# NilanEkanayake/TiTok-Video

Measured on AMD Instinct MI355X. Metric: video clips/sec encode+decode (whole node), higher is better.
Workload: dtype bf16

## Files before the change

include/titok_hip.h:

```cpp
#ifndef TITOK_HIP_H
#define TITOK_HIP_H

#include <stdint.h>

#ifdef __cplusplus
extern "C" {
#endif

#define TTV_OK 0
#define TTV_ERR_INVALID 1
#define TTV_ERR_LAUNCH 2
#define TTV_ERR_UNSUPPORTED 3

#define TTV_BF16 0
#define TTV_F32 1

#define TTV_ENCODER 0
#define TTV_DECODER 1

#define TTV_MAX_FSQ 8
#define TTV_MAX_TOKEN 64
#define TTV_MAX_CLIPS_PER_LAUNCH 64

const char* ttv_error_string(void);
// ... 50 lines not shown

int ttv_rmsnorm(const void* in, int in_dtype, int ld_in, const int32_t* src_rows, void* out, int out_dtype, int ld_out,
                const int32_t* dst_rows, const float* gain, int rows, int width, float eps, void* stream);

int ttv_rope_apply(void* x, int dtype, int ld, int rows, int heads, const float* rope_cs, void* stream);

int ttv_linear(const void* x, int ldx, const void* w, int ldw, const void* bias, const float* add_scalar, void* y, int ldy,
               int M, int N, int K, int dtype, void* stream);

int ttv_linear_qkv_rope(const void* x, int ldx, const void* w, int ldw, void* y, int ldy, int M, int d_model, int gqa_dim,
                        const float* rope_cs, int dtype, void* stream);
int ttv_linear_geglu(const void* x, int ldx, const void* w, int ldw, void* y, int ldy, int M, int I, int K, int dtype,
                     void* stream);
int ttv_linear_residual(const void* x, int ldx, const void* w, int ldw, const void* resid, int ldr, float alpha, void* y,
                        int ldy, int y_f32, int M, int N, int K, int dtype, void* stream);

int ttv_linear_residual_norm(const void* x, int ldx, const void* w, int ldw, const void* resid, int ldr, float alpha,
                             const float* gain, float eps, void* y, int ldy, int M, int N, int K, int dtype, void* stream);

int64_t ttv_mlp_pack_bytes(int inner, int next_qkv_rows);
int ttv_mlp_pack(const void* w12_folded, const void* w3, const void* out_proj, const void* next_qkv_folded, int next_qkv_rows, int inner,
                 int width, int dtype, void* mlp_packed, void* stream);
int ttv_mlp_fused(const void* x, int ldx, const void* mlp_packed, int inner, void* y, int ldy, const float* post_gain, float alpha,
                  float eps, int M, int width, int dtype, void* stream);
typedef struct ttv_next_qkv {
  void* qkv; int32_t ld;
  const float* rope_cs;
  int32_t rows;
  int32_t rope_q_end, rope_k_begin, rope_k_end;
} ttv_next_qkv;
int ttv_layer_tail_fused(const void* ao, int ldao, const float* attn_post_gain, float attn_alpha, const void* x, int ldx,
                         const void* mlp_packed, int inner, void* y, int ldy, const float* ffd_post_gain, float ffd_alpha, float eps,
                         int M, int width, int dtype, const ttv_next_qkv* next, void* stream);

int ttv_fill_const_rows(void* x, int dtype, int ld, const int32_t* rows_map, int rows, int width, const float* mask_token,
                        const float* gain, float eps, void* stream);
int ttv_decoder_embed(const void* codes, int token_size, const void* w, const void* bias, const float* mask_token, const float* gain,
                      void* x, int dtype, int ld, const int32_t* rows_map, int rows, int width, float eps, void* stream);

#define TTV_ATTN_GATE 1
#define TTV_ATTN_PAIRED 2
#define TTV_ATTN_QSCALED 4
#define TTV_ATTN_ALLFULL 8
#define TTV_ATTN_PIPE 16
#define TTV_ATTN_SPLIT3 32
#define TTV_ATTN_SPLIT_OUT 64
#define TTV_ATTN_SPLIT_IN 128
int ttv_attention(const void* qkvg, int ld, void* out, int ldo, const int32_t* cu_seqlens, const int32_t* qblocks,
                  int n_qblocks, int q_heads, int kv_heads, int head_dim, int flags, int dtype, void* stream);
int ttv_attention64(const void* qkvg, int ld, void* out, int ldo, const int32_t* cu_seqlens, const int32_t* items, int n_items,
                    int q_heads, int kv_heads, int head_dim, int flags, int dtype, void* stream);

int ttv_rmsnorm_mx(const void* in, int in_dtype, int ld_in, void* out, int out_dtype, int ld_out, const float* gain, int rows, int width,
                   float eps, float* next_rstd, void* mx_q, void* mx_s, void* stream);
int ttv_attention_mxout(const void* qkvg, int ld, void* out_q, void* out_mx, int ld_mx, const int32_t* cu_seqlens, const int32_t* qblocks,
                        int n_qblocks, int q_heads, int kv_heads, void* stream);
int ttv_linear_fp8_mx_geglu_q(const void* xq, int ldx, const void* x_mx, const float* x_row_scale, const void* wq, int ldw, const void* w_mx,
                              const float* w_row_scale, void* hq, void* hq_mx, int M, int N, int K, void* stream);

int ttv_row_rstd(const void* x, int dtype, int ldx, float* rstd, int rows, int width, float eps, void* stream);
int ttv_linear_rowscale(const void* x, int ldx, const void* w, int ldw, const float* row_scale, int epilogue, const float* rope_cs, int d_model,
                        int gqa_dim, void* y, int ldy, int M, int N, int K, int dtype, void* stream);

int ttv_patch_gather(const void* const* clips, const int32_t* clip_desc, int clip0, int n_clips, int patch_t, int patch_h,
                     int patch_w, int channels, void* patches, int ld, int dtype, int max_patches_per_clip, void* stream);
int ttv_patch_embed_norm(const void* const* clips, const int32_t* clip_desc, const int32_t* patch_rows, const int32_t* row_seq, int n_clips,
                         int patch_t, int patch_h, int patch_w, int channels, const void* w, int ldw, const void* bias,
                         const float* mask_token, const float* gain, float eps, void* x, int ldx, int rows, int width, int dtype,
                         void* stream);
int ttv_patch_scatter(const void* patches, int ld, const int32_t* clip_desc, int clip0, int n_clips, int patch_t, int patch_h,
                      int patch_w, int channels, void* const* clips, int dtype, int max_patches_per_clip, void* stream);
// ... 358 lines not shown
#define TTV_KC_GEMM_RESID 4
#define TTV_KC_GEMM_STORE 5
#define TTV_KC_RMSNORM 6
#define TTV_KC_PATCH 7
#define TTV_KC_ROWS 8
int ttv_prof_begin(int kernel_class, int max_records);
enum {
  TTV_DBG_NO_STORES = 1,
  TTV_DBG_K256_NO_PANEL_DMA = 2,
  TTV_DBG_MLP_NO_WEIGHT_DMA = 2,
  TTV_DBG_K256_NO_TILE_RELOAD = 4,
  TTV_DBG_MLP_NO_GEGLU = 4,
  TTV_DBG_K256_NO_EPILOGUE_MATH = 8,
  TTV_DBG_MLP_TILES8 = 8,
  TTV_DBG_MLP_NO_P2 = 16,
  TTV_DBG_MLP_PAIRS_ONLY = 32,
  TTV_DBG_MLP_TILES4 = 64,
  TTV_DBG_GEMM_TILE160 = 128,
  TTV_DBG_GEMM_TILE128 = 256,
  TTV_DBG_GEMM_T256 = 512,
  TTV_DBG_MLP_TILES9 = 512,
  TTV_DBG_GEMM_NO_T256 = 1024,
  TTV_DBG_MX_UNFUSED_QUANT = 2048,
  TTV_DBG_SPLIT3_NO_IMAGES = 4096,
  TTV_DBG_SPLIT3_NO_DMA = 8192,
  TTV_DBG_K256_GENERAL = 16384,
  TTV_DBG_QKV256_OFF = 32768,
  TTV_DBG_QKV256_WS = 131072,
  TTV_DBG_ENC_ALL_ROWS = 524288,
  TTV_DBG_ATTN_NO_SWP = 1048576,
  TTV_DBG_DEC_ALL_BLOCKS = 2097152,
  TTV_DBG_DEC_L0_NO_CONST = 4194304,
  TTV_DBG_ENC_LAST_QKV_ALL = 8388608,
  TTV_DBG_PATCH_EMBED_UNFUSED = 16777216
};
int ttv_debug_set(int flags);
int ttv_debug_stamps(void* device_buffer);
int ttv_prof_end(double* total_ms, int* count);

#ifdef __cplusplus
}
#endif
#endif
```

titok_video_amd/_lib.py:

```python
from __future__ import annotations

import ctypes as C
import os
import threading

import torch

from . import switches

TTV_BF16, TTV_F32 = 0, 1
TTV_ENCODER, TTV_DECODER = 0, 1
TTV_MAX_FSQ = 8
TTV_MAX_TOKEN = 64
TTV_MAX_CLIPS_PER_LAUNCH = 64
TTV_DISC_HEAD_GENERATOR, TTV_DISC_HEAD_DISCRIMINATOR = 0, 1
TTV_TAPE_STORED, TTV_TAPE_RECOMPUTE = 0, 1

DBG_NO_STORES = 1
DBG_K256_NO_PANEL_DMA = 2
DBG_MLP_NO_WEIGHT_DMA = 2
DBG_K256_NO_TILE_RELOAD = 4
DBG_MLP_NO_GEGLU = 4
DBG_K256_NO_EPILOGUE_MATH = 8
DBG_MLP_TILES8 = 8
DBG_MLP_NO_P2 = 16
DBG_MLP_PAIRS_ONLY = 32
DBG_MLP_TILES4 = 64
DBG_GEMM_TILE160 = 128
DBG_GEMM_TILE128 = 256
DBG_GEMM_T256 = 512
DBG_MLP_TILES9 = 512
DBG_GEMM_NO_T256 = 1024
DBG_MX_UNFUSED_QUANT = 2048
DBG_SPLIT3_NO_IMAGES = 4096
DBG_SPLIT3_NO_DMA = 8192
DBG_K256_GENERAL = 16384
DBG_QKV256_OFF = 32768
DBG_QKV256_WS = 131072
DBG_ENC_ALL_ROWS = 524288
DBG_ATTN_NO_SWP = 1048576
DBG_DEC_ALL_BLOCKS = 2097152
DBG_DEC_L0_NO_CONST = 4194304
DBG_ENC_LAST_QKV_ALL = 8388608
DBG_PATCH_EMBED_UNFUSED = 16777216

_HERE = os.path.dirname(os.path.abspath(__file__))
LIB_PATH = switches.text("TTV_LIB_PATH") or os.path.join(_HERE, "libtitok_hip.so")

i32, i64, f32, vp = C.c_int32, C.c_int64, C.c_float, C.c_void_p


class FsqParams(C.Structure):
    _fields_ = [("n", i32), ("levels", i32 * TTV_MAX_FSQ), ("basis", i32 * TTV_MAX_FSQ),
                ("half_l", f32 * TTV_MAX_FSQ), ("offset", f32 * TTV_MAX_FSQ), ("shift", f32 * TTV_MAX_FSQ),
                ("half_width", f32 * TTV_MAX_FSQ)]


class TowerDims(C.Structure):
    _fields_ = [("kind", i32), ("dtype", i32), ("width", i32), ("layers", i32), ("q_heads", i32), ("kv_heads", i32),
                ("head_dim", i32), ("inner", i32), ("patch_t", i32), ("patch_h", i32), ("patch_w", i32),
                ("pix_channels", i32), ("token_size", i32), ("eps", f32), ("alpha", f32)]


class NextQkv(C.Structure):
    _fields_ = [("qkv", vp), ("ld", i32), ("rope_cs", vp), ("rows", i32), ("rope_q_end", i32), ("rope_k_begin", i32), ("rope_k_end", i32)]


class LayerWeights(C.Structure):
    _fields_ = [("pre_ln", vp), ("to_qkv", vp), ("out_proj", vp), ("ffd_norm", vp), ("w12", vp), ("w3", vp),
                ("attn_post_ln", vp), ("ffd_post_ln", vp), ("to_qkv_pn", vp), ("w12_pn", vp), ("mlp_pack", vp), ("mlp_pack_qkv_rows", i32), ("qkv_q_prescaled", i32),
                ("to_qkv_qs", vp), ("to_qkv_f8", vp), ("to_qkv_f8_scale", vp), ("w12_f8", vp), ("w12_f8_scale", vp),
                ("to_qkv_mx", vp), ("w12_mx", vp), ("out_proj_f8", vp), ("out_proj_f8_scale", vp), ("out_proj_mx", vp),
                ("w3_f8", vp), ("w3_f8_scale", vp), ("w3_mx", vp)]


class TowerWeights(C.Structure):
    _fields_ = [("proj_in_w", vp), ("proj_in_b", vp), ("mask_token", vp), ("ln_pre_t", vp), ("ln_pre_p", vp),
# ... 99 lines not shown
    "ttv_fsq_forward": (C.c_int, [C.POINTER(FsqParams), vp, C.c_int, C.c_int, vp, C.c_int, vp, vp, vp]),
    "ttv_fsq_indices_to_codes": (C.c_int, [C.POINTER(FsqParams), vp, C.c_int, vp, C.c_int, vp]),
    "ttv_vq_codebook_norms": (C.c_int, [vp, C.c_int, C.c_int, C.c_int, C.c_int, vp, vp]),
    "ttv_vq_workspace_bytes": (C.c_int64, [C.c_int]),
    "ttv_vq_l2_argmin": (C.c_int, [vp, C.c_int, C.c_int, vp, C.c_int, vp, C.c_int, C.c_int, C.c_int, vp, vp, vp, C.c_int64, vp]),
    "ttv_vq_lookup": (C.c_int, [vp, C.c_int, C.c_int, vp, C.c_int, C.c_int, vp, C.c_int, vp]),
    "ttv_vq_lookup_backward": (C.c_int, [vp, C.c_int, C.c_int, vp, C.c_int, C.c_int, vp, C.c_int, vp]),
    "ttv_vq_train_workspace_bytes": (C.c_int64, [C.c_int, C.c_int]),
    "ttv_vq_commit_forward": (C.c_int, [vp, C.c_int, C.c_int, vp, C.c_int, vp, C.c_int, C.c_int, C.c_int, vp, vp, C.c_int64, vp]),
    "ttv_vq_commit_backward": (C.c_int, [vp, C.c_int, vp, C.c_int, vp, C.c_int, C.c_int, C.c_int, C.c_int, C.c_double, vp, C.c_int, vp]),
    "ttv_vq_ema_stats": (C.c_int, [vp, C.c_int, C.c_int, vp, C.c_int, C.c_int, C.c_int, vp, f32, C.c_uint64, vp, C.c_int, C.c_int, vp, vp, C.c_int64, vp]),
    "ttv_vq_ema_update": (C.c_int, [vp, vp, vp, vp, vp, C.c_int, vp, vp, C.c_int, C.c_int, f32, f32, f32, f32, vp, C.c_int64, vp]),
    "ttv_quant_rows_fp8": (C.c_int, [vp, C.c_int, C.c_int, vp, f32, vp, C.c_int, vp, C.c_int, C.c_int, vp]),
    "ttv_linear_fp8": (C.c_int, [vp, C.c_int, vp, vp, C.c_int, vp, vp, C.c_int, C.c_int, C.c_int, C.c_int, C.c_int, vp, C.c_int, C.c_int, vp]),
    "ttv_split3_pack": (C.c_int, [vp, C.c_int, vp, C.c_int, C.c_int, C.c_int, vp]),
    "ttv_linear_split3": (C.c_int, [vp, C.c_int, vp, C.c_int, vp, vp, C.c_int, C.c_int, C.c_int, C.c_int, vp]),
    "ttv_mx_scale_bytes_per_row": (C.c_int64, [C.c_int]),
    "ttv_quant_mx_fp8": (C.c_int, [vp, C.c_int, C.c_int, vp, C.c_int, vp, vp, C.c_int, C.c_int, vp]),
    "ttv_linear_fp8_mx": (C.c_int, [vp, C.c_int, vp, vp, vp, C.c_int, vp, vp, vp, C.c_int, C.c_int, C.c_int, C.c_int, C.c_int, vp, C.c_int, C.c_int,
                                    vp, C.c_int, f32, vp]),
    "ttv_rmsnorm": (C.c_int, [vp, C.c_int, C.c_int, vp, vp, C.c_int, C.c_int, vp, vp, C.c_int, C.c_int, f32, vp]),
    "ttv_rope_apply": (C.c_int, [vp, C.c_int, C.c_int, C.c_int, C.c_int, vp, vp]),
    "ttv_linear": (C.c_int, [vp, C.c_int, vp, C.c_int, vp, vp, vp, C.c_int, C.c_int, C.c_int, C.c_int, C.c_int, vp]),
    "ttv_linear_qkv_rope": (C.c_int, [vp, C.c_int, vp, C.c_int, vp, C.c_int, C.c_int, C.c_int, C.c_int, vp, C.c_int, vp]),
    "ttv_linear_geglu": (C.c_int, [vp, C.c_int, vp, C.c_int, vp, C.c_int, C.c_int, C.c_int, C.c_int, C.c_int, vp]),
    "ttv_linear_residual": (C.c_int, [vp, C.c_int, vp, C.c_int, vp, C.c_int, f32, vp, C.c_int, C.c_int, C.c_int, C.c_int,
                                      C.c_int, C.c_int, vp]),
    "ttv_linear_residual_norm": (C.c_int, [vp, C.c_int, vp, C.c_int, vp, C.c_int, f32, vp, f32, vp, C.c_int, C.c_int, C.c_int,
                                           C.c_int, C.c_int, vp]),
    "ttv_mlp_pack_bytes": (C.c_int64, [C.c_int, C.c_int]),
    "ttv_mlp_pack": (C.c_int, [vp, vp, vp, vp, C.c_int, C.c_int, C.c_int, C.c_int, vp, vp]),
    "ttv_layer_tail_fused": (C.c_int, [vp, C.c_int, vp, f32, vp, C.c_int, vp, C.c_int, vp, C.c_int, vp, f32, f32, C.c_int, C.c_int,
                                       C.c_int, vp, vp]),
    "ttv_mlp_fused": (C.c_int, [vp, C.c_int, vp, C.c_int, vp, C.c_int, vp, f32, f32, C.c_int, C.c_int, C.c_int, vp]),
    "ttv_fill_const_rows": (C.c_int, [vp, C.c_int, C.c_int, vp, C.c_int, C.c_int, vp, vp, f32, vp]),
    "ttv_decoder_embed": (C.c_int, [vp, C.c_int, vp, vp, vp, vp, vp, C.c_int, C.c_int, vp, C.c_int, C.c_int, f32, vp]),
    "ttv_attention": (C.c_int, [vp, C.c_int, vp, C.c_int, vp, vp, C.c_int, C.c_int, C.c_int, C.c_int, C.c_int, C.c_int, vp]),
    "ttv_attention64": (C.c_int, [vp, C.c_int, vp, C.c_int, vp, vp, C.c_int, C.c_int, C.c_int, C.c_int, C.c_int, C.c_int, vp]),
    "ttv_rmsnorm_mx": (C.c_int, [vp, C.c_int, C.c_int, vp, C.c_int, C.c_int, vp, C.c_int, C.c_int, f32, vp, vp, vp, vp]),
    "ttv_attention_mxout": (C.c_int, [vp, C.c_int, vp, vp, C.c_int, vp, vp, C.c_int, C.c_int, C.c_int, vp]),
    "ttv_linear_fp8_mx_geglu_q": (C.c_int, [vp, C.c_int, vp, vp, vp, C.c_int, vp, vp, vp, vp, C.c_int, C.c_int, C.c_int, vp]),
    "ttv_row_rstd": (C.c_int, [vp, C.c_int, C.c_int, vp, C.c_int, C.c_int, f32, vp]),
    "ttv_linear_rowscale": (C.c_int, [vp, C.c_int, vp, C.c_int, vp, C.c_int, vp, C.c_int, C.c_int, vp, C.c_int, C.c_int, C.c_int, C.c_int, C.c_int, vp]),
    "ttv_patch_gather": (C.c_int, [C.POINTER(vp), vp, C.c_int, C.c_int, C.c_int, C.c_int, C.c_int, C.c_int, vp, C.c_int,
                                   C.c_int, C.c_int, vp]),
    "ttv_patch_embed_norm": (C.c_int, [C.POINTER(vp), vp, vp, vp, C.c_int, C.c_int, C.c_int, C.c_int, C.c_int, vp, C.c_int, vp, vp, vp, f32,
                                       vp, C.c_int, C.c_int, C.c_int, C.c_int, vp]),
    "ttv_patch_scatter": (C.c_int, [vp, C.c_int, vp, C.c_int, C.c_int, C.c_int, C.c_int, C.c_int, C.c_int, C.POINTER(vp),
                                    C.c_int, C.c_int, vp]),
    "ttv_tower_workspace_bytes": (i64, [C.POINTER(TowerDims), C.POINTER(Batch)]),
    "ttv_encoder_forward": (C.c_int, [C.POINTER(TowerDims), C.POINTER(TowerWeights), C.POINTER(Batch), C.POINTER(vp),
                                      C.POINTER(FsqParams), vp, vp, vp, vp, vp, i64, vp]),
    "ttv_decoder_forward": (C.c_int, [C.POINTER(TowerDims), C.POINTER(TowerWeights), C.POINTER(Batch), vp, C.POINTER(vp),
                                      vp, i64, vp]),
    "ttv_dec_l0_const_bytes": (i64, [C.POINTER(TowerDims), C.c_int]),
    "ttv_dec_l0_const_build": (C.c_int, [C.POINTER(TowerDims), C.POINTER(TowerWeights), vp, vp, vp, vp, C.c_int, vp, i64, C.POINTER(i64), C.POINTER(i64), vp]),
    "ttv_decoder_forward_const": (C.c_int, [C.POINTER(TowerDims), C.POINTER(TowerWeights), C.POINTER(Batch), vp, C.POINTER(vp),
                                            vp, i64, C.POINTER(DecL0Const), vp]),
    "ttv_tower_tape_bytes": (i64, [C.POINTER(TowerDims), C.POINTER(Batch)]),
    "ttv_tower_bwd_workspace_bytes": (i64, [C.POINTER(TowerDims), C.POINTER(Batch)]),
    "ttv_encoder_forward_train": (C.c_int, [C.POINTER(TowerDims), C.POINTER(TowerWeights), C.POINTER(Batch), C.POINTER(vp), vp, vp,
                                            i64, vp]),
    "ttv_encoder_backward": (C.c_int, [C.POINTER(TowerDims), C.POINTER(TowerWeights), C.POINTER(TowerWeightsT), C.POINTER(Batch), vp,
                                       vp, C.POINTER(TowerGrads), C.POINTER(vp), vp, i64, vp]),
    "ttv_decoder_forward_train": (C.c_int, [C.POINTER(TowerDims), C.POINTER(TowerWeights), C.POINTER(Batch), vp, C.POINTER(vp), vp,
                                            i64, vp, i64, vp]),
    "ttv_decoder_backward": (C.c_int, [C.POINTER(TowerDims), C.POINTER(TowerWeights), C.POINTER(TowerWeightsT), C.POINTER(Batch), vp,
                                       C.POINTER(vp), vp, C.POINTER(TowerGrads), vp, vp, i64, vp]),
    "ttv_tower_tape_bytes_ex": (i64, [C.POINTER(TowerDims), C.POINTER(Batch), C.c_int]),
# ... 127 lines not shown
```

titok_video_amd/csrc/ttv_api.hip:

```cpp
#include <stdarg.h>
#include <stdio.h>
#include <stdlib.h>
#include <string.h>

#include "ttv_common.h"
#include "ttv_kernels.h"

static thread_local char g_err[512] = "";

void ttv_set_error(const char* fmt, ...) {
  va_list ap;
  va_start(ap, fmt);
  vsnprintf(g_err, sizeof(g_err), fmt, ap);
  va_end(ap);
}

int g_ttv_prof_class = 0;
bool ttv_sw_enc_latent_last() { static const bool v = ttv_env_flag("TTV_ENC_LATENT_LAST", true); return v; }
bool ttv_enc_latent_rows_only(const ttv_tower_dims* d, const ttv_batch* b) {
  return ttv_sw_enc_latent_last() && !(g_ttv_debug & TTV_DBG_ENC_ALL_ROWS) && d->kind == TTV_ENCODER && b->latent_rows && b->sum_tokens > 0 &&
         b->sum_tokens < b->total_rows;
}
bool ttv_sw_keel_f32sum() { static const bool v = ttv_env_flag("TTV_KEEL_F32SUM", false); return v; }
bool ttv_sw_fused_patch() { static const bool v = ttv_env_flag("TTV_FUSED_PATCH", true); return v; }
bool ttv_sw_attn_pipe() { static const bool v = ttv_env_flag("TTV_ATTN_PIPE", false); return v; }
static bool sw_dec_l0_const() { static const bool v = ttv_env_flag("TTV_DEC_L0_CONST", true); return v; }
static bool sw_enc_last_qkv_skip() { static const bool v = ttv_env_flag("TTV_ENC_LAST_QKV_SKIP", true); return v; }
float ttv_sw_attn_thr() { static const float v = ttv_env_float("TTV_ATTN_THR", 8.0f); return v; }
thread_local int g_ttv_debug = 0;
long long* g_ttv_stamps = nullptr;
static hipEvent_t* g_prof_start = nullptr;
static hipEvent_t* g_prof_stop = nullptr;
static int g_prof_cap = 0, g_prof_n = 0;

TtvProfScope::TtvProfScope(int cls, hipStream_t stream) : slot(-1), s(stream) {
  if (g_ttv_prof_class != 0 && cls == g_ttv_prof_class && g_prof_n < g_prof_cap) {
    slot = g_prof_n++;
    (void)hipEventRecord(g_prof_start[slot], s);
  }
}
TtvProfScope::~TtvProfScope() {
  if (slot >= 0) (void)hipEventRecord(g_prof_stop[slot], s);
}

struct TowerWs {
  char *x, *xn, *qkv, *ao, *h, *pa, *pb;
  char *xl, *aol;
  char *f8, *f8mx;
  float* y32;
  float* rstd;
  int64_t total;
};

static TowerWs carve(const ttv_tower_dims* d, const ttv_batch* b, char* base) {
  const int64_t e = dtype_bytes(d->dtype);
  const int64_t L = b->total_rows, P = b->sum_patches;
  const int64_t g = (int64_t)d->kv_heads * d->head_dim;
  const int64_t pd = patch_dim(d);
  int64_t off = 0;
  TowerWs w;
// ... 74 lines not shown
    TTV_TRY(ttvk_rmsnorm(ws.x, dt, dm, nullptr, ws.x, dt, dm, nullptr, lw.attn_post_ln, L, dm, d->eps, s, ws.rstd, fused_q ? ws.f8 : nullptr,
                         fused_q ? ws.f8mx : nullptr));
    if (!fused_q) TTV_TRY(ttvk_quant_mx_fp8(ws.x, dt, dm, ws.f8, dm, ws.f8mx, nullptr, L, dm, s));
  } else {
    TTV_TRY(ttvk_row_rstd(ws.x, dt, dm, ws.rstd, L, dm, d->eps, s));
    TTV_TRY(ttvk_quant_mx_fp8(ws.x, dt, dm, ws.f8, dm, ws.f8mx, nullptr, L, dm, s));
  }
  GemmArgs f = gemm_args(dt, ws.f8, dm, lw.w12_f8, dm, L, I, dm, ws.h, I);
  char* const hq = ws.h;
  char* const hq_mx = ws.xn;
  const bool h_fused = fused_q && (int64_t)ttvk_mx_scale_ld(I) <= (int64_t)dm * 2;
  if (h_fused) { f.yq = hq; f.yq_mx = hq_mx; }
  TTV_TRY(ttvk_gemm_fp8(EPI_GEGLU, f, ws.rstd, lw.w12_f8_scale, s, ws.f8mx, lw.w12_mx));
  if (!h_fused) TTV_TRY(ttvk_quant_mx_fp8(ws.h, dt, I, ws.f8, I, ws.f8mx, nullptr, L, I, s));
  const GemmArgs f3 = gemm_resid(gemm_args(dt, h_fused ? hq : ws.f8, I, lw.w3_f8, I, L, dm, I, ws.x, dm), ws.x, dm, alpha);
  TTV_TRY(ttvk_gemm_fp8(EPI_RESID_T, f3, nullptr, lw.w3_f8_scale, s, h_fused ? hq_mx : ws.f8mx, lw.w3_mx));
  rstd_valid = false;
  if (i > 0) {
    TTV_TRY(ttvk_rmsnorm(ws.x, dt, dm, nullptr, ws.x, dt, dm, nullptr, lw.ffd_post_ln, L, dm, d->eps, s, ws.rstd, fused_q ? ws.f8 : nullptr,
                         fused_q ? ws.f8mx : nullptr));
    rstd_valid = true;
    xq_valid = fused_q;
  }
  return TTV_OK;
}

static bool rows_f8(int dt, int dm, const void* img, const void* row_scale, const void* mx, const void* folded) {
  return dt == TTV_BF16 && img && row_scale && !mx && dm % 128 == 0 && !(dm == 256 && folded);
}

struct PreNormW { const float* gain; const void *w, *w_pn, *w_f8; const float* w_f8_scale; bool f8; };

static int prenorm_proj(const LayerCtx& c, GemmEpilogue epi, const char* x, int rows, const PreNormW& p, int N, char* y, int y_image,
                        bool rstd_valid, int tile_run = 0, int tile_period = 0, int panel_lo = 0) {
  const ttv_tower_dims* d = c.d;
  const TowerWs& ws = c.ws;
  const int dm = d->width, dt = d->dtype;
  GemmArgs a = gemm_args(dt, nullptr, dm, nullptr, dm, rows, N, dm, y, N);
  if (epi == EPI_QKV_ROPE) a = gemm_rope_qk(a, c.b->rope_cs, dm, d->kv_heads * d->head_dim);
  if (p.f8) {
    float* const f8_scales = reinterpret_cast<float*>(ws.xn + align256((int64_t)c.b->total_rows * dm));
    TTV_TRY(ttvk_quant_rows_fp8(x, dt, dm, p.gain, d->eps, ws.xn, dm, f8_scales, rows, dm, c.s));
    a.x = ws.xn; a.w = p.w_f8;
    return ttvk_gemm_fp8(epi, a, f8_scales, p.w_f8_scale, c.s);
  }
  const bool fold256 = dt == TTV_BF16 && dm == 256 && p.w_pn;
  const bool fold_gen = c.gen_ok && p.w_pn;
  const bool fold = fold256 || fold_gen;
  if (fold_gen && !rstd_valid) TTV_TRY(ttvk_row_rstd(x, dt, dm, ws.rstd, rows, dm, d->eps, c.s));
  if (!fold) TTV_TRY(ttvk_rmsnorm(x, dt, dm, nullptr, ws.xn, dt, dm, nullptr, p.gain, rows, dm, d->eps, c.s, nullptr, nullptr, nullptr, c.s3img));
  a.split3 = c.split3; a.x_image = c.s3img && !fold; a.y_image = y_image;
  a.prenorm = fold256; a.eps = d->eps;
  a.row_scale = fold_gen ? ws.rstd : nullptr;
  a.x = fold ? x : ws.xn; a.w = fold ? p.w_pn : p.w;
  if (epi == EPI_QKV_ROPE) { a.rope_ids = c.b->rope_ids; a.rope_base = c.b->rope_ids ? c.b->rope_base : nullptr; }
  a.tile_run = tile_run; a.tile_period = tile_period; a.panel_lo = panel_lo;
  return ttvk_gemm(epi, a, c.s);
}

static int keel_tail(const LayerCtx& c, GemmArgs o, int layer, const float* post_gain, bool want_rstd, bool& rstd_valid) {
  const ttv_tower_dims* d = c.d;
  const int dm = d->width, dt = d->dtype;
  char* const cx = (char*)o.y;
  o = gemm_resid(o, cx, dm, keel_alpha(d, layer));
  o.split3 = c.split3; o.x_image = c.s3img;
  if (layer == 0) return ttvk_gemm(EPI_RESID_T, o, c.s);
  if (ttvk_gemm_supports_resid_norm(dt, dm, o.K)) {
    o.norm_gain = post_gain; o.eps = d->eps;
    return ttvk_gemm(EPI_RESID_NORM, o, c.s);
  }
  float* const next_rstd = want_rstd ? c.ws.rstd : nullptr;
  if (dt == TTV_BF16 && !ttv_sw_keel_f32sum()) {
    TTV_TRY(ttvk_gemm(EPI_RESID_T, o, c.s));
    TTV_TRY(ttvk_rmsnorm(cx, dt, dm, nullptr, cx, dt, dm, nullptr, post_gain, o.M, dm, d->eps, c.s, next_rstd));
  } else {
    o.y = c.ws.y32;
    TTV_TRY(ttvk_gemm(EPI_RESID_F32, o, c.s));
    TTV_TRY(ttvk_rmsnorm(c.ws.y32, TTV_F32, dm, nullptr, cx, dt, dm, nullptr, post_gain, o.M, dm, d->eps, c.s, next_rstd));
  }
  rstd_valid = want_rstd;
  return TTV_OK;
}

static bool qkv_tile_list_ok(const LayerCtx& c, const ttv_layer_weights& lw, int K, int P) {
  const ttv_tower_dims* d = c.d;
  const ttv_batch* b = c.b;
  if (d->dtype != TTV_BF16 || d->width != 256 || d->head_dim != 64 || c.split3) return false;
  if (K <= 0 || P <= 0 || K % 128 || P % 128 || (int64_t)b->n_clips * K != b->sum_tokens || (int64_t)b->n_clips * P != b->sum_patches) return false;
  if (!lw.to_qkv_pn || !lw.qkv_q_prescaled) return false;
  return ttvk_gemm_qkv_tiles_supported(d->width, d->kv_heads * d->head_dim, d->width);
}

static bool dec_l0_const_ok(const LayerCtx& c, const ttv_tower_weights* w, const ttv_dec_l0_const* l0) {
  const ttv_tower_dims* d = c.d;
  const ttv_batch* b = c.b;
  if (!l0 || !l0->rows || !sw_dec_l0_const() || (g_ttv_debug & TTV_DBG_DEC_L0_NO_CONST)) return false;
  if (d->kind != TTV_DECODER || !qkv_tile_list_ok(c, w->layers[0], l0->latent_rows, l0->patch_rows)) return false;
  if (c.pair || c.pipe || !c.all_full || (b->items64 && b->n_items64 > 0)) return false;
  return ttvk_attention_takes_swp(TTV_ATTN_GATE | TTV_ATTN_QSCALED | TTV_ATTN_ALLFULL);
}

static bool enc_last_qkv_skip_ok(const LayerCtx& c, const ttv_layer_weights& lw) {
  const ttv_batch* b = c.b;
  if (!sw_enc_last_qkv_skip() || (g_ttv_debug & TTV_DBG_ENC_LAST_QKV_ALL) || c.d->kind != TTV_ENCODER) return false;
  return qkv_tile_list_ok(c, lw, b->tokens_per_clip, b->max_patches_per_clip);
}

static int run_layers(const ttv_tower_dims* d, const ttv_tower_weights* w, const ttv_batch* b, const TowerWs& ws, hipStream_t s,
                      const ttv_dec_l0_const* l0 = nullptr) {
  const int L = b->total_rows, dm = d->width, g = d->kv_heads * d->head_dim, dt = d->dtype;
  const int split3 = (dt == TTV_F32 && w->f32_split3) ? 1 : 0;
  const bool gen_ok = (dt == TTV_BF16 && dm != 256) || split3;
  static const bool s3img_env = ttv_env_flag("TTV_SPLIT3_IMAGES", true);
  const int s3img = (split3 && s3img_env && !(g_ttv_debug & TTV_DBG_SPLIT3_NO_IMAGES)) ? 1 : 0;
  const int nq = 2 * dm + 2 * g;
  const int64_t row_bytes = (int64_t)dm * dtype_bytes(dt);
  bool qkv_ready = false;
  bool rstd_valid = false;
  bool xq_valid = false;
  const bool lat_last = ttv_enc_latent_rows_only(d, b) && b->qblocks_latent && b->n_qblocks_latent > 0;
  static const bool pat_env = ttv_env_flag("TTV_DEC_PATCH_LAST", true);
  const bool pat_last = pat_env && !(g_ttv_debug & TTV_DBG_DEC_ALL_BLOCKS) && d->kind == TTV_DECODER && d->layers >= 2 && b->qblocks_patch &&
                        b->n_qblocks_patch > 0 && !split3 && !b->qblocks_paired;
  bool compacted = false;
  const LayerCtx ctx = {d, b, ws, s, split3, s3img, gen_ok, b->qblocks_paired ? TTV_ATTN_PAIRED : 0, b->qblocks_all_full ? TTV_ATTN_ALLFULL : 0,
                        ttv_sw_attn_pipe() ? TTV_ATTN_PIPE : 0};
  const bool l0_const = dec_l0_const_ok(ctx, w, l0);
  for (int i = 0; i < d->layers; ++i) {
    const ttv_layer_weights& lw = w->layers[i];
    const bool last = i == d->layers - 1;
    const bool l0c = l0_const && i == 0;
    if (dt == TTV_BF16 && dm != 256 && dm % 128 == 0 && d->inner % 128 == 0 && !ttv_sw_keel_f32sum() && lw.to_qkv_f8 && lw.to_qkv_mx && lw.w12_f8 &&
        lw.w12_mx && lw.out_proj_f8 && lw.out_proj_mx && lw.w3_f8 && lw.w3_mx &&
        !(lat_last && last)) {
      TTV_TRY(run_layer_mx(ctx, lw, i, rstd_valid, xq_valid));
      qkv_ready = false;
      continue;
    }
    xq_valid = false;
    const bool f8_qkv = rows_f8(dt, dm, lw.to_qkv_f8, lw.to_qkv_f8_scale, lw.to_qkv_mx, lw.to_qkv_pn);
    const bool f8_w12 = rows_f8(dt, dm, lw.w12_f8, lw.w12_f8_scale, lw.w12_mx, lw.w12_pn);
    if (!qkv_ready) {
      const void* w_plain = (dt == TTV_BF16 && lw.to_qkv_qs) ? lw.to_qkv_qs : lw.to_qkv;
      const PreNormW qw = {lw.pre_ln, w_plain, lw.to_qkv_pn, lw.to_qkv_f8, lw.to_qkv_f8_scale, f8_qkv};
      if (l0c) TTV_TRY(prenorm_proj(ctx, EPI_QKV_ROPE, ws.x, L, qw, nq, ws.qkv, 0, rstd_valid, l0->latent_rows / 128, (l0->latent_rows + l0->patch_rows) / 128));
      else if (lat_last && last && !f8_qkv && enc_last_qkv_skip_ok(ctx, lw))
        TTV_TRY(prenorm_proj(ctx, EPI_QKV_ROPE, ws.x, L, qw, nq, ws.qkv, 0, rstd_valid, b->tokens_per_clip / 128,
                             (b->tokens_per_clip + b->max_patches_per_clip) / 128, 2 * dm / 64));
      else TTV_TRY(prenorm_proj(ctx, EPI_QKV_ROPE, ws.x, L, qw, nq, ws.qkv, s3img ? 2 : 0, rstd_valid));
    }
    const bool q_scaled = dt == TTV_BF16 && (lw.to_qkv_pn ? lw.qkv_q_prescaled != 0 : lw.to_qkv_qs != nullptr);
    rstd_valid = false;
    qkv_ready = false;
    const bool lat_now = lat_last && last;
    if (lat_now)
      TTV_TRY(tower_attention(ctx, q_scaled, b->qblocks_latent, b->n_qblocks_latent, ctx.all_full));
    else if (l0c) {
      TtvProfScope prof(TTV_KC_ATTENTION, s);
      const bool own = l0->qblocks && l0->n_qblocks > 0;
      TTV_TRY(ttvk_attention_swp(ws.qkv, nq, ws.ao, dm, b->cu_seqlens, own ? l0->qblocks : b->qblocks, own ? l0->n_qblocks : b->n_qblocks, d->q_heads,
                                 d->kv_heads, 1, s, l0->rows, l0->latent_rows, l0->state));
    } else if (pat_last && last && dt == TTV_BF16 && !ctx.pipe)
      TTV_TRY(tower_attention(ctx, q_scaled, b->qblocks_patch, b->n_qblocks_patch, ctx.all_full));
    else if (q_scaled && b->items64 && b->n_items64 > 0 && d->head_dim == 64)
      TTV_TRY(ttvk_attention64(ws.qkv, nq, ws.ao, dm, b->cu_seqlens, b->items64, b->n_items64, d->q_heads, d->kv_heads,
                               TTV_ATTN_GATE | TTV_ATTN_QSCALED, s));
    else
      TTV_TRY(tower_attention(ctx, q_scaled, b->qblocks, b->n_qblocks, ctx.pair | ctx.all_full | ctx.pipe));
    char* cx = ws.x;
    char* cao = ws.ao;
    int Lc = L;
    if (lat_now) {
      TTV_TRY(gather_rows(ws.x, ws.xl, b->latent_rows, b->sum_tokens, row_bytes, s));
      TTV_TRY(gather_rows(ws.ao, ws.aol, b->latent_rows, b->sum_tokens, row_bytes, s));
      cx = ws.xl; cao = ws.aol; Lc = b->sum_tokens;
      compacted = true;
    }
    static const bool use_fused_mlp = ttv_env_flag("TTV_FUSED_MLP", true);
    static const bool use_fused_qkv = ttv_env_flag("TTV_FUSED_QKV", false);
    const float alpha = keel_alpha(d, i);
    if (use_fused_mlp && ttvk_mlp_fused_supported(dt, dm, d->inner) && lw.mlp_pack) {
      MlpNextQkv nx = {};
      const bool back = use_fused_qkv && !last && lw.mlp_pack_qkv_rows == nq && nq % 64 == 0 && dm % 64 == 0 && g % 64 == 0;
      if (back) { nx.qkv = ws.qkv; nx.ld = nq; nx.rope_cs = b->rope_cs; nx.rows = nq; nx.rope_q_end = dm; nx.rope_k_begin = 2 * dm; nx.rope_k_end = 2 * dm + g; }
      TTV_TRY(ttvk_mlp_fused(cao, dm, i == 0 ? nullptr : lw.attn_post_ln, alpha, cx, dm, lw.mlp_pack, d->inner, cx, dm, i == 0 ? nullptr : lw.ffd_post_ln,
                             alpha, d->eps, Lc, back ? &nx : nullptr, s));
      qkv_ready = back;
      continue;
    }
    TTV_TRY(keel_tail(ctx, gemm_args(dt, cao, dm, lw.out_proj, dm, Lc, dm, dm, cx, dm), i, lw.attn_post_ln, gen_ok && lw.w12_pn && !f8_w12, rstd_valid));
    const PreNormW fw = {lw.ffd_norm, lw.w12, lw.w12_pn, lw.w12_f8, lw.w12_f8_scale, f8_w12};
    TTV_TRY(prenorm_proj(ctx, EPI_GEGLU, cx, Lc, fw, d->inner, ws.h, s3img, rstd_valid));
    rstd_valid = false;
    const ttv_layer_weights* nl = last ? nullptr : &w->layers[i + 1];
    const bool next_rstd = gen_ok && nl && nl->to_qkv_pn && !rows_f8(dt, dm, nl->to_qkv_f8, nl->to_qkv_f8_scale, nl->to_qkv_mx, nl->to_qkv_pn);
    TTV_TRY(keel_tail(ctx, gemm_args(dt, ws.h, d->inner, lw.w3, d->inner, Lc, dm, d->inner, cx, dm), i, lw.ffd_post_ln, next_rstd, rstd_valid));
  }
  if (compacted)
    TTV_TRY(scatter_rows(ws.xl, ws.x, b->latent_rows, b->sum_tokens, row_bytes, s));
  return TTV_OK;
}

static bool fused_patch_ok(const ttv_tower_dims* d, const ttv_batch* b, int dt) {
  auto pow2 = [](int v) { return v > 0 && (v & (v - 1)) == 0; };
  return ttv_sw_fused_patch() && dt == TTV_BF16 && d->patch_w == 8 && pow2(d->patch_t) && pow2(d->patch_h) &&
         b->n_clips <= TTV_MAX_CLIPS_PER_LAUNCH && b->row_seq && patch_dim(d) % 64 == 0;
}

extern "C" {

const char* ttv_error_string(void) { return g_err; }
int ttv_version(void) { return 100; }

int ttv_fsq_forward(const ttv_fsq_params* p, const void* z, int z_dtype, int rows, void* codes, int codes_dtype, int32_t* indices,
                    float* bounded, void* stream) {
  TTV_CHECK_ARG(rows >= 0 && (rows == 0 || (z && codes && indices)), "fsq_forward: null buffer");
  return ttvk_fsq_forward(p, z, z_dtype, rows, codes, codes_dtype, indices, bounded, (hipStream_t)stream);
}

// ... 169 lines not shown
int ttv_mlp_pack(const void* w12_folded, const void* w3, const void* out_proj, const void* next_qkv_folded, int next_qkv_rows, int inner,
                 int width, int dtype, void* packed, void* stream) {
  if (!ttvk_mlp_fused_supported(dtype, width, inner)) {
    ttv_set_error("mlp_pack: only bf16, width 256, inner %% 32 == 0");
    return TTV_ERR_UNSUPPORTED;
  }
  return ttvk_mlp_pack(w12_folded, w3, out_proj, next_qkv_folded, next_qkv_rows, inner, packed, (hipStream_t)stream);
}

int ttv_mlp_fused(const void* x, int ldx, const void* mlp_packed, int inner, void* y, int ldy, const float* post_gain, float alpha,
                  float eps, int M, int width, int dtype, void* stream) {
  if (!ttvk_mlp_fused_supported(dtype, width, inner)) {
    ttv_set_error("mlp_fused: only bf16, width 256, inner %% 32 == 0");
    return TTV_ERR_UNSUPPORTED;
  }
  return ttvk_mlp_fused(nullptr, 0, nullptr, 1.f, x, ldx, mlp_packed, inner, y, ldy, post_gain, alpha, eps, M, nullptr, (hipStream_t)stream);
}

int ttv_layer_tail_fused(const void* ao, int ldao, const float* attn_post_gain, float attn_alpha, const void* x, int ldx,
                         const void* mlp_packed, int inner, void* y, int ldy, const float* ffd_post_gain, float ffd_alpha, float eps,
                         int M, int width, int dtype, const ttv_next_qkv* next, void* stream) {
  if (!ttvk_mlp_fused_supported(dtype, width, inner)) {
    ttv_set_error("layer_tail_fused: only bf16, width 256, inner %% 32 == 0");
    return TTV_ERR_UNSUPPORTED;
  }
  TTV_CHECK_ARG(ao, "layer_tail_fused: null attention output");
  MlpNextQkv nx = {};
  if (next) { nx.qkv = next->qkv; nx.ld = next->ld; nx.rope_cs = next->rope_cs; nx.rows = next->rows; nx.rope_q_end = next->rope_q_end;
              nx.rope_k_begin = next->rope_k_begin; nx.rope_k_end = next->rope_k_end; }
  return ttvk_mlp_fused(ao, ldao, attn_post_gain, attn_alpha, x, ldx, mlp_packed, inner, y, ldy, ffd_post_gain, ffd_alpha, eps, M,
                        next ? &nx : nullptr, (hipStream_t)stream);
}

int ttv_fill_const_rows(void* x, int dtype, int ld, const int32_t* rows_map, int rows, int width, const float* mask_token,
                        const float* gain, float eps, void* stream) {
  TTV_CHECK_ARG(rows == 0 || (x && rows_map && mask_token && gain), "fill_const_rows: null buffer");
  return ttvk_fill_const_rows(x, dtype, ld, rows_map, rows, width, mask_token, gain, eps, (hipStream_t)stream);
}

int ttv_decoder_embed(const void* codes, int token_size, const void* w, const void* bias, const float* mask_token, const float* gain,
                      void* x, int dtype, int ld, const int32_t* rows_map, int rows, int width, float eps, void* stream) {
  TTV_CHECK_ARG(rows == 0 || (codes && w && bias && mask_token && gain && x && rows_map), "decoder_embed: null buffer");
  return ttvk_dec_embed(codes, token_size, w, bias, mask_token, gain, x, dtype, ld, rows_map, rows, width, eps, (hipStream_t)stream);
}

int ttv_attention(const void* qkvg, int ld, void* out, int ldo, const int32_t* cu_seqlens, const int32_t* qblocks, int n_qblocks,
                  int q_heads, int kv_heads, int head_dim, int flags, int dtype, void* stream) {
  TTV_CHECK_ARG(n_qblocks == 0 || (qkvg && out && cu_seqlens && qblocks), "attention: null buffer");
  return ttvk_attention(qkvg, ld, out, ldo, cu_seqlens, qblocks, n_qblocks, q_heads, kv_heads, head_dim, flags, dtype, (hipStream_t)stream);
}
int ttv_attention64(const void* qkvg, int ld, void* out, int ldo, const int32_t* cu_seqlens, const int32_t* items, int n_items, int q_heads,
                    int kv_heads, int head_dim, int flags, int dtype, void* stream) {
  TTV_CHECK_ARG(dtype == TTV_BF16 && head_dim == 64, "attention64: bf16, head_dim 64 only");
  return ttvk_attention64(qkvg, ld, out, ldo, cu_seqlens, items, n_items, q_heads, kv_heads, flags, (hipStream_t)stream);
}

int ttv_rmsnorm_mx(const void* in, int in_dtype, int ld_in, void* out, int out_dtype, int ld_out, const float* gain, int rows, int width,
                   float eps, float* next_rstd, void* mx_q, void* mx_s, void* stream) {
  TTV_CHECK_ARG(rows >= 0 && (rows == 0 || (in && out && gain)), "rmsnorm_mx: null buffer");
  TTV_CHECK_ARG(!mx_q == !mx_s, "rmsnorm_mx: the image needs both its element and its scale buffer");
  return ttvk_rmsnorm(in, in_dtype, ld_in, nullptr, out, out_dtype, ld_out, nullptr, gain, rows, width, eps, (hipStream_t)stream, next_rstd, mx_q, mx_s);
}

int ttv_attention_mxout(const void* qkvg, int ld, void* out_q, void* out_mx, int ld_mx, const int32_t* cu_seqlens, const int32_t* qblocks,
                        int n_qblocks, int q_heads, int kv_heads, void* stream) {
  TTV_CHECK_ARG(n_qblocks >= 0 && (n_qblocks == 0 || (qkvg && out_q && out_mx && cu_seqlens && qblocks)), "attention_mxout: null buffer");
  return ttvk_attention_mxout(qkvg, ld, out_q, out_mx, ld_mx, cu_seqlens, qblocks, n_qblocks, q_heads, kv_heads, (hipStream_t)stream);
}

int ttv_linear_fp8_mx_geglu_q(const void* xq, int ldx, const void* x_mx, const float* x_row_scale, const void* wq, int ldw, const void* w_mx,
                              const float* w_row_scale, void* hq, void* hq_mx, int M, int N, int K, void* stream) {
  TTV_CHECK_ARG(M == 0 || (xq && wq && x_mx && w_mx && hq && hq_mx), "linear_fp8_mx_geglu_q: null buffer");
  GemmArgs a = gemm_args(TTV_BF16, xq, ldx, wq, ldw, M, N, K, hq, N);
  a.yq = hq; a.yq_mx = hq_mx;
  return ttvk_gemm_fp8(EPI_GEGLU, a, x_row_scale, w_row_scale, (hipStream_t)stream, x_mx, w_mx);
}
// ... 116 lines not shown
  char* const rows = (char*)block;
  const int64_t state_floats = ttvk_attention_swp_state_floats(patch_rows, d->q_heads);
  float* const state = (float*)(rows + align256((int64_t)patch_rows * nq * 2));
  char* const x = (char*)state + align256(state_floats * 4 + 4);
  if (state_offset) *state_offset = (char*)state - rows;
  if (flag_offset) *flag_offset = (char*)(state + state_floats) - rows;
  TTV_TRY(ttvk_fill_const_rows(x, dt, dm, iota, patch_rows, dm, w->mask_token, w->ln_pre_p, d->eps, s));
  GemmArgs a = gemm_rope_qk(gemm_args(dt, x, dm, lw.to_qkv_pn, dm, patch_rows, nq, dm, rows, nq), rope_cs, dm, g);
  a.prenorm = 1; a.eps = d->eps;
  a.rope_ids = rope_ids; a.rope_base = rope_ids ? rope_base : nullptr;
  TTV_TRY(ttvk_gemm(EPI_QKV_ROPE, a, s));
  if (hipMemsetAsync(state + state_floats, 0, 4, s) != hipSuccess) {
    ttv_set_error("dec_l0_const_build: hipMemsetAsync failed");
    return TTV_ERR_LAUNCH;
  }
  return ttvk_attention_swp_dump(rows, nq, patch_rows, d->q_heads, d->kv_heads, state, s);
}

int ttv_decoder_forward(const ttv_tower_dims* d, const ttv_tower_weights* w, const ttv_batch* b, const void* codes,
                        void* const* clips_out, void* workspace, int64_t workspace_bytes, void* stream) {
  return ttv_decoder_forward_const(d, w, b, codes, clips_out, workspace, workspace_bytes, nullptr, stream);
}

int ttv_decoder_forward_const(const ttv_tower_dims* d, const ttv_tower_weights* w, const ttv_batch* b, const void* codes,
                              void* const* clips_out, void* workspace, int64_t workspace_bytes, const ttv_dec_l0_const* l0, void* stream) {
  TTV_TRY(check_dims(d, b));
  TTV_CHECK_ARG(d->kind == TTV_DECODER, "decoder_forward: dims.kind is not TTV_DECODER");
  TTV_CHECK_ARG(w && w->layers && codes && clips_out && workspace, "decoder_forward: null argument");
  hipStream_t s = (hipStream_t)stream;
  TowerWs ws = carve(d, b, (char*)workspace);
  TTV_CHECK_ARG(ws.total <= workspace_bytes, "decoder_forward: workspace too small (%lld < %lld)", (long long)workspace_bytes, (long long)ws.total);
  const int dm = d->width, dt = d->dtype, P = b->sum_patches, pd = patch_dim(d);

  TTV_TRY(ttvk_dec_embed(codes, d->token_size, w->proj_in_w, w->proj_in_b, w->mask_token, w->ln_pre_t, ws.x, dt, dm, b->latent_rows, b->sum_tokens, dm, d->eps, s));
  TTV_TRY(ttvk_fill_const_rows(ws.x, dt, dm, b->patch_rows, P, dm, w->mask_token, w->ln_pre_p, d->eps, s));

  TTV_TRY(run_layers(d, w, b, ws, s, l0));

  GemmArgs a = gemm_args(dt, nullptr, dm, w->proj_out_w, dm, P, pd, dm, ws.pa, pd);
  a.split3 = (dt == TTV_F32 && w->f32_split3) ? 1 : 0;
  a.bias = w->proj_out_b;
  if (dt == TTV_BF16 && dm == 256 && w->proj_out_pn && pd % 8 == 0) {
    a.x = ws.x; a.x_rows = b->patch_rows; a.w = w->proj_out_pn; a.prenorm = 1; a.eps = d->eps;
  } else {
    TTV_TRY(ttvk_rmsnorm(ws.x, dt, dm, b->patch_rows, ws.pb, dt, dm, nullptr, w->ln_post, P, dm, d->eps, s));
    a.x = ws.pb;
  }
  if (fused_patch_ok(d, b, dt) && dm == 256) {
    a.clips = clips_out; a.n_clips = b->n_clips; a.clip_desc = b->clip_desc; a.patch_rows = b->patch_rows; a.row_seq = b->row_seq;
    a.patch_t = d->patch_t; a.patch_h = d->patch_h; a.patch_w = d->patch_w;
    return ttvk_gemm(EPI_STORE_PATCH, a, s);
  }
  TTV_TRY(ttvk_gemm(EPI_STORE, a, s));
  return patch_copy_all(true, clips_out, d, b, ws.pa, dt, s);
}

int ttv_rope_table_build(const float* base_cos, const float* base_sin, int n_ids, int n_freqs, const int32_t* clip_desc, const int32_t* cu_seqlens,
                         const int32_t* row_seq, float* rope_cs, int total_rows, void* stream) {
  TTV_CHECK_ARG(total_rows == 0 || (base_cos && base_sin && clip_desc && cu_seqlens && row_seq && rope_cs), "rope_table_build: null buffer");
  TTV_CHECK_ARG(n_freqs >= 1 && 3 * n_freqs <= 32 && n_ids >= 1, "rope_table_build: bad table shape");
  return ttvk_rope_build(base_cos, base_sin, n_ids, n_freqs, clip_desc, cu_seqlens, row_seq, rope_cs, total_rows, (hipStream_t)stream);
}

int ttv_l1_loss(void* const* recon, void* const* target, void* const* grad, const int32_t* sizes, int n_clips, int dtype, float* loss,
                void* stream) {
  return for_clip_groups(n_clips, [&](int c0, int n) {
    return ttvk_l1_loss(recon + c0, target + c0, grad ? grad + c0 : nullptr, sizes + c0, n, n_clips, dtype, loss, (hipStream_t)stream);
  });
// ... 178 lines not shown
```

titok_video_amd/csrc/ttv_elem.hip:

```cpp
#include "ttv_common.h"
#include "ttv_kernels.h"

#define ROWS_PER_BLOCK 4
#define MAX_ITERS 4

__device__ __forceinline__ int mx_quant4(const f32x4 y, int& byte) {
  float a = fmaxf(fmaxf(fabsf(y[0]), fabsf(y[1])), fmaxf(fabsf(y[2]), fabsf(y[3])));
  a = fmaxf(a, __shfl_xor(a, 1));
  a = fmaxf(a, __shfl_xor(a, 2));
  a = fmaxf(a, __shfl_xor(a, 4));
  const uint32_t tb = __float_as_uint(a * (1.0f / 448.0f));
  byte = (int)((tb >> 23) & 0xFF) + ((tb & 0x7FFFFF) ? 1 : 0);
  byte = a > 0.f ? (byte < 1 ? 1 : (byte > 254 ? 254 : byte)) : 127;
  const float inv_blk = __uint_as_float((uint32_t)(254 - byte) << 23);
  int w = 0;
  w = __builtin_amdgcn_cvt_pk_fp8_f32(y[0] * inv_blk, y[1] * inv_blk, w, false);
  w = __builtin_amdgcn_cvt_pk_fp8_f32(y[2] * inv_blk, y[3] * inv_blk, w, true);
  return w;
}

template <typename TI, typename TO>
__global__ __launch_bounds__(256) void k_rmsnorm(const TI* __restrict__ in, int ld_in, const int* __restrict__ src_rows,
                                                 TO* __restrict__ out, int ld_out, const int* __restrict__ dst_rows,
                                                 const float* __restrict__ gain, int rows, int d, float eps,
// ... 305 lines not shown
    a = fmaxf(a, __shfl_xor(a, 2));
    a = fmaxf(a, __shfl_xor(a, 4));
    const uint32_t tb = __float_as_uint(a * (1.0f / 448.0f));
    int byte = (int)((tb >> 23) & 0xFF) + ((tb & 0x7FFFFF) ? 1 : 0);
    byte = a > 0.f ? (byte < 1 ? 1 : (byte > 254 ? 254 : byte)) : 127;
    const float inv_blk = __uint_as_float((uint32_t)(254 - byte) << 23);
    int w = 0;
    w = __builtin_amdgcn_cvt_pk_fp8_f32(y[0] * inv_blk, y[1] * inv_blk, w, false);
    w = __builtin_amdgcn_cvt_pk_fp8_f32(y[2] * inv_blk, y[3] * inv_blk, w, true);
    *reinterpret_cast<int*>(q + c) = w;
    if ((lane & 7) == 0) {
      const int b = c >> 5;
      m[(b & 3) * nkp + (b >> 2)] = (uint8_t)byte;
    }
  }
}

int64_t ttvk_mx_scale_ld(int d) { return 4 * (int64_t)((d / 128 + 3) / 4 * 4); }

int ttvk_quant_mx_fp8(const void* in, int in_dtype, int ld_in, void* out, int ld_out, void* mx, float* row_scales, int rows, int d, hipStream_t s) {
  if (rows == 0) return TTV_OK;
  TTV_CHECK_ARG(d > 0 && d % 128 == 0, "quant_mx_fp8: width %d must be a multiple of 128", d);
  TTV_CHECK_ARG(ld_in % 4 == 0 && ld_out % 4 == 0 && (uintptr_t)out % 4 == 0 && (uintptr_t)mx % 4 == 0, "quant_mx_fp8: alignment");
  const int nkp = (d / 128 + 3) / 4 * 4;
  dim3 grid(ttv_cdiv(rows, ROWS_PER_BLOCK));
  if (in_dtype == TTV_BF16) hipLaunchKernelGGL((k_quant_mx_fp8<bf16_t>), grid, dim3(256), 0, s, (const bf16_t*)in, ld_in, (uint8_t*)out, ld_out, (uint8_t*)mx, 4 * nkp, nkp, row_scales, rows, d);
  else if (in_dtype == TTV_F32) hipLaunchKernelGGL((k_quant_mx_fp8<float>), grid, dim3(256), 0, s, (const float*)in, ld_in, (uint8_t*)out, ld_out, (uint8_t*)mx, 4 * nkp, nkp, row_scales, rows, d);
  else { ttv_set_error("quant_mx_fp8: bad dtype"); return TTV_ERR_INVALID; }
  TTV_CHECK_LAUNCH("quant_mx_fp8");
  return TTV_OK;
}

template <typename T>
__global__ __launch_bounds__(256) void k_fill_const_rows(T* __restrict__ x, int ld, const int* __restrict__ rows_map, int rows,
                                                         int d, const float* __restrict__ mask_token,
                                                         const float* __restrict__ gain, float eps) {
  const int wave = threadIdx.x >> 6, lane = threadIdx.x & 63;
  const int r = blockIdx.x * ROWS_PER_BLOCK + wave;
  if (r >= rows) return;
  const float m = round_to<T>(mask_token[0]);
  const float rstd = 1.0f / sqrtf(m * m + eps);
  T* q = x + (size_t)rows_map[r] * ld;
  for (int c = lane * 4; c < d; c += 256) {
    const f32x4 g = *reinterpret_cast<const f32x4*>(gain + c);
    f32x4 o = {m * rstd * g[0], m * rstd * g[1], m * rstd * g[2], m * rstd * g[3]};
    Vec4<T>::store(q + c, o);
  }
}

int ttvk_fill_const_rows(void* x, int dtype, int ld, const int* rows_map, int rows, int d, const float* mask_token,
                         const float* gain, float eps, hipStream_t s) {
  if (rows == 0) return TTV_OK;
  TTV_CHECK_ARG(d % 4 == 0, "fill_const_rows: width %% 4");
  dim3 grid(ttv_cdiv(rows, ROWS_PER_BLOCK));
  if (dtype == TTV_BF16)
    hipLaunchKernelGGL((k_fill_const_rows<bf16_t>), grid, dim3(256), 0, s, (bf16_t*)x, ld, rows_map, rows, d, mask_token, gain, eps);
  else
    hipLaunchKernelGGL((k_fill_const_rows<float>), grid, dim3(256), 0, s, (float*)x, ld, rows_map, rows, d, mask_token, gain, eps);
  TTV_CHECK_LAUNCH("fill_const_rows");
  return TTV_OK;
}

template <typename T>
__global__ __launch_bounds__(256) void k_dec_embed(const T* __restrict__ codes, int C, const T* __restrict__ w ,
                                                   const T* __restrict__ bias, const float* __restrict__ mask_token,
                                                   const float* __restrict__ gain, T* __restrict__ x, int ld,
                                                   const int* __restrict__ rows_map, int rows, int d, float eps, T* __restrict__ hpre) {
  const int wave = threadIdx.x >> 6, lane = threadIdx.x & 63;
  const int r = blockIdx.x * ROWS_PER_BLOCK + wave;
  if (r >= rows) return;
  float cz[TTV_MAX_FSQ];
#pragma unroll
  for (int c = 0; c < TTV_MAX_FSQ; ++c) cz[c] = c < C ? Cvt<T>::to_f(codes[(size_t)r * C + c]) : 0.f;
  const T* crow = codes + (size_t)r * C;
  const float m = round_to<T>(mask_token[0]);
  float v[MAX_ITERS][4];
  float ss = 0.f;
#pragma unroll
  for (int it = 0; it < MAX_ITERS; ++it) {
#pragma unroll
    for (int e = 0; e < 4; ++e) {
      const int f = (it * 64 + lane) * 4 + e;
      float h = 0.f;
      if (f < d) {
        if (C <= TTV_MAX_FSQ) {
#pragma unroll
          for (int c = 0; c < TTV_MAX_FSQ; ++c)
            if (c < C) h += cz[c] * Cvt<T>::to_f(w[(size_t)f * C + c]);
        } else if ((C & 3) == 0) {
          const T* wrow = w + (size_t)f * C;
          for (int c = 0; c < C; c += 4) {
            const f32x4 cv = Vec4<T>::load(crow + c), wv = Vec4<T>::load(wrow + c);
            h += cv[0] * wv[0];
            h += cv[1] * wv[1];
            h += cv[2] * wv[2];
            h += cv[3] * wv[3];
          }
        } else {
          for (int c = 0; c < C; ++c) h += Cvt<T>::to_f(crow[c]) * Cvt<T>::to_f(w[(size_t)f * C + c]);
        }
        h = round_to<T>(h + Cvt<T>::to_f(bias[f]));
        h = round_to<T>(h + m);
      }
      v[it][e] = h;
      ss += h * h;
    }
    if (hpre && (it * 64 + lane) * 4 < d)
      Vec4<T>::store(hpre + (size_t)r * d + (it * 64 + lane) * 4, (f32x4){v[it][0], v[it][1], v[it][2], v[it][3]});
  }
  ss = wave_sum(ss);
  const float rstd = 1.0f / sqrtf(ss / (float)d + eps);
  T* q = x + (size_t)rows_map[r] * ld;
#pragma unroll
  for (int it = 0; it < MAX_ITERS; ++it) {
    const int c0 = (it * 64 + lane) * 4;
    if (c0 < d) {
      const f32x4 g = *reinterpret_cast<const f32x4*>(gain + c0);
      f32x4 o = {v[it][0] * rstd * g[0], v[it][1] * rstd * g[1], v[it][2] * rstd * g[2], v[it][3] * rstd * g[3]};
      Vec4<T>::store(q + c0, o);
    }
  }
}

int ttvk_dec_embed(const void* codes, int C, const void* w, const void* bias, const float* mask_token, const float* gain,
                   void* x, int dtype, int ld, const int* rows_map, int rows, int d, float eps, hipStream_t s) {
  return ttvk_dec_embed_ex(codes, C, w, bias, mask_token, gain, x, dtype, ld, rows_map, rows, d, eps, nullptr, s);
}

int ttvk_dec_embed_ex(const void* codes, int C, const void* w, const void* bias, const float* mask_token, const float* gain, void* x,
                      int dtype, int ld, const int* rows_map, int rows, int d, float eps, void* hpre, hipStream_t s) {
  if (rows == 0) return TTV_OK;
  TTV_CHECK_ARG(C >= 1 && C <= TTV_MAX_TOKEN, "dec_embed: token_size %d out of range", C);
  TTV_CHECK_ARG(d % 4 == 0 && d <= 1024, "dec_embed: width");
  dim3 grid(ttv_cdiv(rows, ROWS_PER_BLOCK));
  if (dtype == TTV_BF16)
    hipLaunchKernelGGL((k_dec_embed<bf16_t>), grid, dim3(256), 0, s, (const bf16_t*)codes, C, (const bf16_t*)w, (const bf16_t*)bias, mask_token, gain, (bf16_t*)x, ld, rows_map, rows, d, eps, (bf16_t*)hpre);
  else
    hipLaunchKernelGGL((k_dec_embed<float>), grid, dim3(256), 0, s, (const float*)codes, C, (const float*)w, (const float*)bias, mask_token, gain, (float*)x, ld, rows_map, rows, d, eps, (float*)hpre);
  TTV_CHECK_LAUNCH("dec_embed");
  return TTV_OK;
}

struct FsqDev {
  int n;
  float half_l[TTV_MAX_FSQ], offset[TTV_MAX_FSQ], shift[TTV_MAX_FSQ], half_width[TTV_MAX_FSQ], basis[TTV_MAX_FSQ];
  int levels[TTV_MAX_FSQ], ibasis[TTV_MAX_FSQ];
};

static FsqDev to_dev(const ttv_fsq_params* p) {
  FsqDev d;
  d.n = p->n;
  for (int i = 0; i < TTV_MAX_FSQ; ++i) {
    d.half_l[i] = p->half_l[i]; d.offset[i] = p->offset[i]; d.shift[i] = p->shift[i];
    d.half_width[i] = p->half_width[i]; d.basis[i] = (float)p->basis[i];
// ... 357 lines not shown
```

titok_video_amd/csrc/ttv_gemm.hip:

```cpp
#include <stdlib.h>

#include "ttv_common.h"
#include "ttv_kernels.h"

struct GemmDev {
  const void* x; const void* w; void* y;
  const void* bias; const float* add_scalar; const void* resid; const float* rope_cs;
  int ldx, ldw, ldy, ldr;
  int M, N, K;
  int w_rows;
  float alpha;
  int rope_q_end, rope_k_begin, rope_k_end;
  float eps;
  int debug;
  const float* norm_gain;
  ClipPtrs clips;
  const int* clip_desc; const int* patch_rows; const int* row_seq;
  const int* x_rows;
  const float* row_scale;
  const int* rope_ids; const float* rope_base;
  const float* x_scale; const float* w_scale;
  float* sum_f32; int ld_sum;
  void* y2; int ldy2; const float* norm_gain2;
  int split3;
  int x_image, y_image;
  const uint8_t* x_mx; const uint8_t* w_mx;
  int ld_mx;
  uint8_t* yq; uint8_t* yq_mx; int ld_yq_mx, yq_nkp;
  int clip0, pt_shift, ph_shift;
  long long* stamps;
  int resid_rows;
  int tile_run, tile_period;
  int panel_lo;
};

struct PatchDst {
  bf16_t* base;
  int thw, hw, w;
};

__device__ __forceinline__ float gelu_erf(float v) { return 0.5f * v * (1.0f + erff(v * 0.70710678118654752440f)); }
__device__ __forceinline__ float gelu_erf_as(float v) {
  const float x = fabsf(v) * 0.70710678118654752440f;
  const float t = __builtin_amdgcn_rcpf(fmaf(0.3275911f, x, 1.0f));
  const float poly = t * fmaf(t, fmaf(t, fmaf(t, fmaf(t, 1.061405429f, -1.453152027f), 1.421413741f), -0.284496736f), 0.254829592f);
  const float e = __builtin_amdgcn_exp2f(x * x * -1.44269504088896340736f);
  const float erf_abs = fmaf(-poly, e, 1.0f);
  return 0.5f * v * (1.0f + __builtin_copysignf(erf_abs, v));
}

__device__ __forceinline__ uint2 pack_bf16x4(f32x4 v) {
  bf16x4 b = {(bf16_t)v[0], (bf16_t)v[1], (bf16_t)v[2], (bf16_t)v[3]};
  return __builtin_bit_cast(uint2, b);
}

__device__ __forceinline__ uint4 split4_bf16(uint4 v) {
  const float x0 = __uint_as_float(v.x), x1 = __uint_as_float(v.y), x2 = __uint_as_float(v.z), x3 = __uint_as_float(v.w);
  const bf16_t h0 = (bf16_t)x0, h1 = (bf16_t)x1, h2 = (bf16_t)x2, h3 = (bf16_t)x3;
  const bf16_t l0 = (bf16_t)(x0 - (float)h0), l1 = (bf16_t)(x1 - (float)h1), l2 = (bf16_t)(x2 - (float)h2), l3 = (bf16_t)(x3 - (float)h3);
  const bf16x4 hv = {h0, h1, h2, h3}, lv = {l0, l1, l2, l3};
  const uint2 hp = __builtin_bit_cast(uint2, hv), lp = __builtin_bit_cast(uint2, lv);
  return make_uint4(hp.x, hp.y, lp.x, lp.y);
}

template <int EPI, typename T, int NI, int NJ>
__device__ __forceinline__ void epilogue_tile(const GemmDev& p, const int (&tok)[NJ], const int (&feat)[NI],
// ... 1761 lines not shown
    for (int i = 0; i < 2; ++i) {
      feat[i] = fbase + wf * 32 + i * 16 + kq * 4;
#pragma unroll
      for (int j = 0; j < NJ; ++j) { ax[i][j] = acc[i][j]; ag[i][j] = acc[i + 2][j]; }
    }
    epilogue_tile<EPI, float, 2, NJ>(p, tok, feat, ax, ag, kq);
  } else {
    int feat[4];
#pragma unroll
    for (int i = 0; i < 4; ++i) feat[i] = fbase + wf * 64 + i * 16 + kq * 4;
    epilogue_tile<EPI, float, 4, NJ>(p, tok, feat, acc, acc, kq);
  }
}

static int gemm_token_tile(int M, int nf, int debug) {
  if (debug & TTV_DBG_GEMM_TILE160) return 160;
  if (debug & TTV_DBG_GEMM_TILE128) return 128;
  const long cost128 = (long)ttv_cdiv(nf * ttv_cdiv(M, 128), 512) * 128, cost160 = (long)ttv_cdiv(nf * ttv_cdiv(M, 160), 512) * 160;
  return cost160 < cost128 ? 160 : 128;
}

static int sw_qkv256() { static const int v = ttv_env_int("TTV_QKV256", 1); return v; }
bool ttvk_gemm_qkv_tiles_supported(int d_model, int gqa_dim, int ldw) {
  const int N = 2 * d_model + 2 * gqa_dim;
  return sw_qkv256() == 1 && !(g_ttv_debug & (TTV_DBG_QKV256_OFF | TTV_DBG_QKV256_WS)) && N % 64 == 0 && d_model % 64 == 0 && gqa_dim % 64 == 0 &&
         (uint64_t)N * (uint64_t)ldw * 2u < (1ull << 32);
}

template <int EPI>
static int launch(const GemmDev& d, int dtype, bool prenorm, hipStream_t s) {
  if (dtype == TTV_BF16 && d.K == 256 && d.N % 8 == 0 && !((d.debug & TTV_DBG_K256_GENERAL) && !prenorm && EPI != EPI_STORE_PATCH)) {
    const int fo = (EPI == EPI_GEGLU) ? 32 : 64;
    const int n_panels = ttv_cdiv(d.N, fo), n_tiles = d.tile_period ? d.M / K256_TT / d.tile_period * d.tile_run : ttv_cdiv(d.M, K256_TT);
    const int total = n_panels * n_tiles + (d.panel_lo ? d.M / K256_TT / d.tile_period * (d.tile_period - d.tile_run) * (n_panels - d.panel_lo) : 0);
    static const int grid_env = ttv_env_int("TTV_K256_GRID", 0);
    int grid = total < 512 ? total : 512;
    if (grid_env > 0) grid = total < grid_env ? total : grid_env;
    else if (d.panel_lo && total > 512) {
      const int w = n_panels - d.panel_lo;
      for (int ipb = 2; ipb <= w; ++ipb)
        if (w % ipb == 0 && n_panels % ipb == 0 && total / ipb <= 512) { grid = total / ipb; break; }
    } else if (total > 512)
      for (int g = 512; g >= 416; --g)
        if (total % g == 0) { grid = g; break; }
    const int qkv256_env = sw_qkv256();
    if constexpr (EPI == EPI_QKV_ROPE) {
      const int n_groups = (n_panels + 3) / 4;
      if (qkv256_env && !(d.debug & TTV_DBG_QKV256_OFF) && d.N % 64 == 0 && d.rope_q_end % 64 == 0 && d.rope_k_begin % 64 == 0 && d.rope_k_end % 64 == 0 &&
          !d.row_scale && !d.bias && !d.add_scalar && (uint64_t)d.w_rows * (uint64_t)d.ldw * 2u < (1ull << 32)) {
        if ((qkv256_env >= 2 || (d.debug & TTV_DBG_QKV256_WS)) && n_groups <= 32 && !d.tile_period) {
          const int tgs = ttv_cdiv(d.M, 32), per_xcd = ttv_cdiv(tgs, 8);
          int q = n_groups * ttv_cdiv(per_xcd, 8);
          q = q > 32 ? 32 : q;
          if (prenorm) hipLaunchKernelGGL((k_qkv256ws<true>), dim3(8 * q), dim3(512), 0, s, d, n_panels, n_groups);
          else hipLaunchKernelGGL((k_qkv256ws<false>), dim3(8 * q), dim3(512), 0, s, d, n_panels, n_groups);
          TTV_CHECK_LAUNCH("qkv256ws");
          return TTV_OK;
        }
        if (d.panel_lo) {
          if (prenorm) hipLaunchKernelGGL((k_qkv256<true, true>), dim3(grid), dim3(256), 0, s, d, n_panels, total);
          else hipLaunchKernelGGL((k_qkv256<false, true>), dim3(grid), dim3(256), 0, s, d, n_panels, total);
        } else if (prenorm) hipLaunchKernelGGL((k_qkv256<true, false>), dim3(grid), dim3(256), 0, s, d, n_panels, total);
        else hipLaunchKernelGGL((k_qkv256<false, false>), dim3(grid), dim3(256), 0, s, d, n_panels, total);
        TTV_CHECK_LAUNCH("qkv256");
        return TTV_OK;
      }
    }
    if (d.tile_period) {
      ttv_set_error("gemm: a tile list needs k_qkv256 (ttvk_gemm_qkv_tiles_supported)");
      return TTV_ERR_UNSUPPORTED;
    }
    if (prenorm) hipLaunchKernelGGL((k_gemm_k256<EPI, true>), dim3(grid), dim3(256), 0, s, d, n_panels, total);
    else hipLaunchKernelGGL((k_gemm_k256<EPI, false>), dim3(grid), dim3(256), 0, s, d, n_panels, total);
    TTV_CHECK_LAUNCH("gemm_k256");
    return TTV_OK;
  }
  if (prenorm || EPI == EPI_STORE_PATCH) {
    ttv_set_error("gemm: folded pre-norm / patch scatter need the bf16 K=256 kernel");
    return TTV_ERR_UNSUPPORTED;
  }
  if (dtype == TTV_BF16) {
    const int ft = (EPI == EPI_GEGLU) ? 64 : TF;
    const int nf = ttv_cdiv(d.N, ft), nt = ttv_cdiv(d.M, TT), nt160 = ttv_cdiv(d.M, 160);
    const bool t160 = gemm_token_tile(d.M, nf, d.debug) == 160;
    static const bool use_dma = ttv_env_flag("TTV_GEMM_DMA", true);
    const bool dma_ok = use_dma && d.K % BK == 0 && (uint64_t)d.M * (uint64_t)d.ldx * 2u < (1ull << 32) && (uint64_t)d.w_rows * (uint64_t)d.ldw * 2u < (1ull << 32);
    static const int t256_env = ttv_env_int("TTV_GEMM_T256", -1);
    if constexpr (EPI == EPI_STORE || EPI == EPI_QKV_ROPE || EPI == EPI_GEGLU || EPI == EPI_RESID_T || EPI == EPI_RESID_F32) {
      const int fo = (EPI == EPI_GEGLU) ? 128 : T256_F;
      const long tiles256 = (long)ttv_cdiv(d.N, fo) * ttv_cdiv(d.M, T256_T);
      const bool forced = (d.debug & TTV_DBG_GEMM_T256) || t256_env == 1;
      const bool ok256 = dma_ok && d.N % fo == 0 && d.K >= 2 * BK && !(d.debug & TTV_DBG_GEMM_NO_T256) && (forced || tiles256 >= 256);
// ... 87 lines not shown

bool ttvk_gemm_supports_resid_norm(int dtype, int N, int K) { return dtype == TTV_BF16 && N == 256 && K % 8 == 0; }

int ttvk_gemm(GemmEpilogue epi, const GemmArgs& a, hipStream_t s) {
  if (a.M == 0 || a.N == 0) return TTV_OK;
  const int esz = dtype_bytes(a.dtype);
  const int vec = 16 / esz;
  TTV_CHECK_ARG(a.dtype == TTV_BF16 || a.dtype == TTV_F32, "gemm: bad dtype %d", a.dtype);
  TTV_CHECK_ARG(a.K > 0 && a.K % vec == 0, "gemm: K=%d must be a multiple of %d", a.K, vec);
  TTV_CHECK_ARG(a.N % 4 == 0, "gemm: N=%d must be a multiple of 4", a.N);
  TTV_CHECK_ARG(a.ldx % vec == 0 && a.ldw % vec == 0 && a.ldy % vec == 0, "gemm: leading dims must keep 16-byte row alignment");
  TTV_CHECK_ARG(((uintptr_t)a.x % 16 == 0) && ((uintptr_t)a.w % 16 == 0) && ((uintptr_t)a.y % 16 == 0), "gemm: pointers must be 16-byte aligned");
  GemmDev d;
  d.x = a.x; d.w = a.w; d.y = a.y; d.bias = a.bias; d.add_scalar = a.add_scalar; d.resid = a.resid; d.rope_cs = a.rope_cs; d.rope_ids = a.rope_ids; d.rope_base = a.rope_base;
  d.ldx = a.ldx; d.ldw = a.ldw; d.ldy = a.ldy; d.ldr = a.ldr;
  d.M = a.M; d.N = a.N; d.K = a.K; d.alpha = a.alpha;
  d.w_rows = (epi == EPI_GEGLU) ? 2 * a.N : a.N;
  d.rope_q_end = a.rope_q_end; d.rope_k_begin = a.rope_k_begin; d.rope_k_end = a.rope_k_end;
  d.eps = a.eps;
  d.debug = g_ttv_debug;
  d.sum_f32 = a.sum_f32; d.ld_sum = a.ld_sum; d.y2 = a.y2; d.ldy2 = a.ldy2; d.norm_gain2 = a.norm_gain2;
  d.split3 = (a.split3 && a.dtype == TTV_F32) ? 1 : 0;
  d.x_image = d.split3 && a.x_image; d.y_image = d.split3 ? a.y_image : 0;
  TTV_CHECK_ARG(!d.y_image || (d.y_image == 1 && (epi == EPI_STORE || epi == EPI_GEGLU)) || (d.y_image == 2 && epi == EPI_QKV_ROPE),
                "gemm: a split-image output is a STORE / GEGLU option (y_image 1) or the to_qkv layout (y_image 2)");
  d.x_mx = d.w_mx = nullptr; d.ld_mx = 0;
  d.norm_gain = a.norm_gain;
  d.clip_desc = a.clip_desc; d.patch_rows = a.patch_rows; d.row_seq = a.row_seq; d.clip0 = 0; d.pt_shift = d.ph_shift = 0;
  d.x_rows = a.x_rows;
  d.x_scale = nullptr; d.w_scale = nullptr;
  d.row_scale = a.row_scale;
  d.stamps = g_ttv_stamps;
  d.resid_rows = a.resid_rows;
  d.tile_run = d.tile_period = d.panel_lo = 0;
  TTV_CHECK_ARG(a.panel_lo >= 0 && (!a.panel_lo || (a.tile_period && a.N % 64 == 0 && a.panel_lo < a.N / 64)),
                "gemm: a panel floor goes with a tile list and leaves at least one 64-feature panel");
  if (a.tile_period) {
    TTV_CHECK_ARG(epi == EPI_QKV_ROPE && a.dtype == TTV_BF16 && a.K == 256 && a.tile_run > 0 && a.tile_run < a.tile_period &&
                  a.M % (K256_TT * a.tile_period) == 0, "gemm: a tile list is a to_qkv option of the bf16 K=256 kernel, M a whole number of periods");
    d.tile_run = a.tile_run; d.tile_period = a.tile_period; d.panel_lo = a.panel_lo;
  }
  TTV_CHECK_ARG(!a.row_scale || ((a.dtype == TTV_BF16 || a.split3) && (epi == EPI_STORE || epi == EPI_QKV_ROPE || epi == EPI_GEGLU)),
                "gemm: row_scale is a STORE / QKV_ROPE / GEGLU option of the bf16 and the split-bf16 kernels");
  TTV_CHECK_ARG(!a.x_rows || (a.dtype == TTV_BF16 && a.K == 256 && a.N % 8 == 0 && epi != EPI_RESID_NORM), "gemm: x_rows needs the bf16 K=256 kernel");
  if (epi == EPI_STORE_PATCH || a.gather) {
    auto lg2 = [](int v) { int s = 0; while ((1 << s) < v) ++s; return (1 << s) == v ? s : -1; };
    TTV_CHECK_ARG(a.dtype == TTV_BF16 && (a.gather || a.K == 256) && a.patch_w == 8 && lg2(a.patch_t) >= 0 && lg2(a.patch_h) >= 0,
                  "gemm: patch gather/scatter needs bf16, patch_w == 8 and power-of-two patch_t / patch_h (scatter: K == 256)");
    TTV_CHECK_ARG(!a.gather || (epi == EPI_STORE && a.K % 64 == 0 && a.K != 256), "gemm: patch gather is an EPI_STORE option of the general-K kernel");
    TTV_CHECK_ARG(a.clips && a.n_clips > 0 && a.n_clips <= TTV_MAX_CLIPS_PER_LAUNCH && a.clip_desc && a.patch_rows && a.row_seq,
                  "gemm: patch scatter needs clips (<= %d), clip_desc, patch_rows and row_seq", TTV_MAX_CLIPS_PER_LAUNCH);
    for (int i = 0; i < a.n_clips; ++i) d.clips.p[i] = a.clips[i];
    d.pt_shift = lg2(a.patch_t); d.ph_shift = lg2(a.patch_h);
  }
  const bool pn = a.prenorm != 0;
  const int kc = (epi == EPI_STORE || epi == EPI_STORE_PATCH) ? TTV_KC_GEMM_STORE : epi == EPI_QKV_ROPE ? TTV_KC_GEMM_QKV : epi == EPI_GEGLU ? TTV_KC_GEMM_GEGLU : TTV_KC_GEMM_RESID;
  TtvProfScope prof(kc, s);
  switch (epi) {
    case EPI_STORE:
      if (a.gather) {
        const int nf = ttv_cdiv(d.N, TF), nt = ttv_cdiv(d.M, TT), nt160 = ttv_cdiv(d.M, 160);
        if (gemm_token_tile(d.M, nf, d.debug) == 160)
          hipLaunchKernelGGL((k_gemm_bf16<EPI_STORE, true, 5>), dim3(nf * nt160), dim3(256), 0, s, d, nf);
        else
          hipLaunchKernelGGL((k_gemm_bf16<EPI_STORE, true>), dim3(nf * nt), dim3(256), 0, s, d, nf);
        TTV_CHECK_LAUNCH("gemm_gather");
        return TTV_OK;
      }
      return launch<EPI_STORE>(d, a.dtype, pn, s);
    case EPI_STORE_PATCH: return launch<EPI_STORE_PATCH>(d, a.dtype, pn, s);
    case EPI_QKV_ROPE:
      TTV_CHECK_ARG(a.rope_cs && a.rope_q_end % 128 == 0 && a.rope_k_begin % 128 == 0 && a.rope_k_end % 128 == 0, "gemm: rotary ranges must be multiples of 128 columns");
      return launch<EPI_QKV_ROPE>(d, a.dtype, pn, s);
// ... 52 lines not shown
```

titok_video_amd/csrc/ttv_kernels.h:

```cpp
#pragma once
#include <hip/hip_runtime.h>
#include <stdint.h>

#include "../../include/titok_hip.h"

int ttvk_rmsnorm(const void* in, int in_dtype, int ld_in, const int* src_rows, void* out, int out_dtype, int ld_out,
                 const int* dst_rows, const float* gain, int rows, int d, float eps, hipStream_t s, float* next_rstd = nullptr,
                 void* mx_q = nullptr, void* mx_s = nullptr,
                 int split_image = 0);
int ttvk_row_rstd(const void* in, int dtype, int ld_in, float* rstd, int rows, int d, float eps, hipStream_t s);
int ttvk_copy_rows(const void* src, int64_t ld_src_bytes, const int* src_rows, void* dst, int64_t ld_dst_bytes, const int* dst_rows, int rows,
                   int row_bytes, hipStream_t s);
int ttvk_fill_const_rows(void* x, int dtype, int ld, const int* rows_map, int rows, int d, const float* mask_token,
                         const float* gain, float eps, hipStream_t s);
int ttvk_dec_embed(const void* codes, int C, const void* w, const void* bias, const float* mask_token, const float* gain,
                   void* x, int dtype, int ld, const int* rows_map, int rows, int d, float eps, hipStream_t s);
int ttvk_fsq_forward(const ttv_fsq_params* p, const void* z, int z_dtype, int rows, void* codes, int codes_dtype, int* indices,
                     float* bounded, hipStream_t s);
int ttvk_fsq_indices_to_codes(const ttv_fsq_params* p, const int* indices, int rows, void* codes, int codes_dtype, hipStream_t s);
int ttvk_enc_tail(const void* x, int dtype, int ld, const int* rows_map, int rows, int d, const float* gain, float eps,
                  const void* w, const void* bias, int C, const ttv_fsq_params* fsq, float* z_out, void* codes, int* indices,
                  float* bounded, hipStream_t s);
int ttvk_patch_copy(bool scatter, void* const* clips, const int* clip_desc, int clip0, int n_clips, int pt, int ph, int pw,
                    int C, void* patches, int ld, int dtype, int max_patches, hipStream_t s);
int ttvk_rope_apply(void* x, int dtype, int ld, int rows, int heads, const float* cs, hipStream_t s);
int ttvk_histogram(const int* idx, int n, int64_t* counts, int size, hipStream_t s);
int ttvk_quant_rows_fp8(const void* in, int in_dtype, int ld_in, const float* gain, float eps, void* out, int ld_out, float* scales, int rows,
                        int d, hipStream_t s);

int ttvk_split3_pack(const float* w, int ldw, void* out, int ldo, int rows, int K, hipStream_t s);
int64_t ttvk_mx_scale_ld(int d);
int ttvk_quant_mx_fp8(const void* in, int in_dtype, int ld_in, void* out, int ld_out, void* mx, float* row_scales, int rows, int d, hipStream_t s);

int ttvk_clip_from_u8(const void* frames, long long n_pix, void* clip, int dtype, hipStream_t s);

int ttvk_clip_resample_u8(void* const* src, void* const* dst, const int32_t* geom, int n_clips, int dtype, hipStream_t s);

enum GemmEpilogue {
  EPI_STORE = 0,
  EPI_QKV_ROPE,
  EPI_GEGLU,
  EPI_RESID_T,
  EPI_RESID_F32,
  EPI_RESID_NORM,
  EPI_STORE_PATCH,
  EPI_BIAS_PLAIN,
  EPI_BIAS_GELU,
  EPI_BIAS_RESID_F32R,
};
// ... 1 lines not shown
struct GemmArgs {
  const void* x; int ldx;
  const void* w; int ldw;
  int M, N, K;
  void* y; int ldy;
  const void* bias;
  const float* add_scalar;
  const void* resid; int ldr;
  float alpha;
  const float* rope_cs;
  const int* rope_ids; const float* rope_base;
  int rope_q_end, rope_k_begin, rope_k_end;
  int dtype;
  const float* norm_gain;
  float* sum_f32; int ld_sum;
  void* y2; int ldy2; const float* norm_gain2;
  void* yq; void* yq_mx;
  int split3;
  int x_image, y_image;
  int prenorm;
  const float* row_scale;
  const int* x_rows;
  float eps;
  int gather;
  void* const* clips;
  int n_clips;
  const int* clip_desc;
  const int* patch_rows;
  const int* row_seq;
  int patch_t, patch_h, patch_w;
  int resid_rows;
  int tile_run, tile_period;
  int panel_lo;
};
struct ClipPtrs { void* p[TTV_MAX_CLIPS_PER_LAUNCH]; };
int ttvk_gemm(GemmEpilogue epi, const GemmArgs& a, hipStream_t s);
int ttvk_gemm_fp8(GemmEpilogue epi, const GemmArgs& a, const float* x_scale, const float* w_scale, hipStream_t s, const void* x_mx = nullptr,
                  const void* w_mx = nullptr);
bool ttvk_gemm_supports_resid_norm(int dtype, int N, int K);
bool ttvk_gemm_qkv_tiles_supported(int d_model, int gqa_dim, int ldw);

bool ttvk_patch_embed_norm_supported(int dtype, int width, int patch_dim, int patch_w);
int ttvk_patch_embed_norm(void* const* clips, int clip0, int n_clips, const int* clip_desc, const int* patch_rows, const int* row_seq,
                          int patch_t, int patch_h, int patch_w, int patch_dim, const void* w, int ldw, const void* bias,
                          const float* mask_token, const float* gain, float eps, void* x, int ldx, int M, hipStream_t s);

int ttvk_attention(const void* qkvg, int ld, void* out, int ldo, const int* cu_seqlens, const int* qblocks, int n_qblocks,
                   int q_heads, int kv_heads, int head_dim, int flags, int dtype, hipStream_t s, float* lse_out = nullptr,
                   void* out_raw = nullptr);

bool ttvk_attention_takes_swp(int flags);
int ttvk_attention_swp(const void* qkvg, int ld, void* out, int ldo, const int* cu_seqlens, const int* qblocks, int n_qblocks,
                       int q_heads, int kv_heads, int gate_mul, hipStream_t s, const void* rows2 = nullptr, int kwin = 0,
                       const float* state = nullptr);
int64_t ttvk_attention_swp_state_floats(int n_rows, int q_heads);
int ttvk_attention_swp_dump(const void* rows, int ld, int n_rows, int q_heads, int kv_heads, float* state, hipStream_t s);
int ttvk_attention_mxout(const void* qkvg, int ld, void* out_q, void* out_mx, int ld_mx, const int* cu_seqlens, const int* qblocks,
                         int n_qblocks, int q_heads, int kv_heads, hipStream_t s);

int ttvk_attention64(const void* qkvg, int ld, void* out, int ldo, const int* cu_seqlens, const int* items, int n_items, int q_heads,
                     int kv_heads, int flags, hipStream_t s);

int ttvk_vq_norms(const void* cb, int dtype, int ld, int N, int C, float* cnorm, hipStream_t s);
int64_t ttvk_vq_workspace_bytes(int rows);
int ttvk_vq_l2_argmin(const void* z, int dtype, int ldz, const void* cb, int ldc, const float* cnorm, int rows, int N, int C, int* indices,
                      float* best_dist, void* workspace, int64_t workspace_bytes, hipStream_t s);
int ttvk_vq_lookup(const void* cb, int dtype, int ldc, const int* indices, int rows, int C, void* codes, int ldo, hipStream_t s);
int ttvk_vq_lookup_bwd(const void* dcodes, int dtype, int ld, const int* indices, int rows, int C, float* dcb, int ldc, hipStream_t s);

int64_t ttvk_vq_train_workspace_bytes(int rows, int N);
int ttvk_vq_commit_forward(const void* z, int dtype, int ldz, const void* cb, int ldc, const int* idx, int rows, int N, int C, float* loss,
                           void* workspace, int64_t workspace_bytes, hipStream_t s);
int ttvk_vq_commit_backward(const void* g, int ldg, const void* z, int ldz, const void* e, int lde, int dtype, int rows, int C, double scale,
                            void* dz, int ldd, hipStream_t s);
int ttvk_vq_ema_stats(const void* z, int dtype, int ldz, const int* idx, int rows, int N, int C, const float* cluster_size, float dead_threshold,
                      uint64_t seed, const int64_t* ema_step, int rank, int world_size, float* stats, void* workspace, int64_t workspace_bytes,
                      hipStream_t s);
int ttvk_vq_ema_update(const float* stats, float* cluster_size, float* embed_avg, float* codebook, void* copy, int copy_dtype, float* cnorm,
                       int64_t* ema_step, int N, int C, float decay, float one_minus_decay, float eps, float dead_threshold, void* workspace,
                       int64_t workspace_bytes, hipStream_t s);

bool ttvk_mlp_fused_supported(int dtype, int width, int inner);
struct MlpNextQkv {
  void* qkv; int ld;
  const float* rope_cs;
  int rows;
  int rope_q_end, rope_k_begin, rope_k_end;
};
int64_t ttvk_mlp_pack_bytes(int inner, int next_qkv_rows);
int ttvk_mlp_pack(const void* w12_folded, const void* w3, const void* wo, const void* next_qkv_folded, int next_qkv_rows, int inner,
                  void* packed, hipStream_t s);
int ttvk_mlp_fused(const void* ao, int ldao, const float* front_gain, float front_alpha, const void* x, int ldx, const void* packed,
                   int inner, void* y, int ldy, const float* post_gain, float alpha, float eps, int M, const MlpNextQkv* nq, hipStream_t s);

int ttvk_l1_loss(void* const* recon, void* const* target, void* const* grad, const int* sizes, int n_clips, int total_clips, int dtype,
                 float* loss, hipStream_t s);
int ttvk_sq_err(void* const* recon, void* const* target, const int* sizes, int n_clips, int dtype, int clamp, double* acc2, hipStream_t s);
int ttvk_rmsnorm_bwd_chain(const void* x, int ldx, const void* dy, int lddy, const float* gain1, float* dgain1, float* dx, int lddx,
                           const void* y, int y_dt, int ldy, const float* gain2, float* dgain2, float out_scale, void* cast_out, int ldc, int rows,
                           int d, float eps, int dt, hipStream_t s);
int ttvk_rmsnorm_bwd(const void* x, int x_dt, int ldx, const int* xr, const void* dy, int dy_dt, int lddy, const int* dyr,
                     const float* gain, void* dx, int dx_dt, int lddx, const int* dxr, int acc, float* dgain, int rows, int d, float eps,
                     hipStream_t s);
int ttvk_colsum(const void* a, int dt, int lda, const int* rows_map, int rows, int n, float* out, hipStream_t s);
int ttvk_sumall(const void* a, int dt, int lda, const int* rows_map, int rows, int n, const float* colw, float scale, float* out, hipStream_t s);
int ttvk_gate_fwd(const void* a, int lda, const void* gate, int ldg, void* ag, int ldo, int rows, int d, int dt, hipStream_t s);
int ttvk_gate_bwd(const void* dag, int ldd, const void* a, int lda, const void* gate, int ldg, void* da, int ldda, void* dgate, int lddg,
                  int rows, int d, int dt, float* delta, hipStream_t s);
int ttvk_geglu_fwd(const void* u, int ldu, void* h, int ldh, int rows, int I, int dt, hipStream_t s);
int ttvk_geglu_bwd(const void* u, int ldu, const void* dh, int lddh, void* du, int lddu, int rows, int I, int dt, hipStream_t s);
int ttvk_scale_cast(const float* a, float alpha, float* b, void* c, int dt, long n, hipStream_t s);
int ttvk_to_f32(const void* a, int dt, float* b, long n, int accumulate, hipStream_t s);
int ttvk_fsq_bwd(const ttv_fsq_params* fp, const float* z, const void* dcodes, int dt, float* dz, int rows, hipStream_t s);
#define TTV_WGRAD_BATCH 6
struct WgradBatch {
  int n = 0;
  int64_t used_bytes = 0;
  struct Entry { const float* part; float* dw; int splits, lddw, N, K, tiles_n, tiles; } e[TTV_WGRAD_BATCH];
};
int ttvk_wgrad(const void* dy, int lddy, const void* x, int ldx, float* dw, int lddw, int L, int N, int K, int dt, float* part,
               int64_t part_bytes, hipStream_t s, WgradBatch* batch = nullptr);
int ttvk_wgrad_flush(WgradBatch* batch, hipStream_t s);
int64_t ttvk_wgrad_ws_bytes(int L, int N, int K);
int ttvk_outer_small(const void* a, int a_dt, int lda, int C, const void* b, int b_dt, int ldb, const int* b_rows, float* dw, int lddw,
                     int transpose_out, int rows, int d, hipStream_t s);
int ttvk_expand_small(const void* a, int a_dt, int lda, int C, const void* w, int w_dt, int ldw, int w_cf, void* out, int o_dt, int ldo,
// ... 102 lines not shown
```

titok_video_amd/csrc/ttv_mlp.hip:

```cpp
#include "ttv_common.h"
#include "ttv_kernels.h"

#define MLP_W12_CHUNKS 2048
#define MLP_W3_CHUNKS 1024
#define MLP_PANEL_CHUNKS (MLP_W12_CHUNKS + MLP_W3_CHUNKS)
#define MLP_WO_CHUNKS (4 * MLP_W12_CHUNKS)

struct MlpDev {
  const bf16_t* x; int ldx;
  const uint4* pack;
  const bf16_t* ao; int ldao;
  const float* front_gain;
  float front_alpha;
  bf16_t* qkv; int ldq;
  const float* rope_cs;
  int nqp, rope_q_end, rope_k_begin, rope_k_end;
  int I;
  bf16_t* y; int ldy;
  const float* post_gain;
  float alpha, eps;
  int M, n_tiles, debug;
  long long* stamps;
};

__global__ void k_mlp_pack(const bf16_t* __restrict__ w12f, const bf16_t* __restrict__ w3, const bf16_t* __restrict__ wo,
                           const bf16_t* __restrict__ wq, int nq_rows, int I, uint4* __restrict__ out) {
  const int np = I / 32;
  const int nqp = (nq_rows + 63) / 64;
  const int o = blockIdx.x * blockDim.x + threadIdx.x;
  if (o >= np * MLP_PANEL_CHUNKS + MLP_WO_CHUNKS + nqp * MLP_W12_CHUNKS) return;
  if (o >= np * MLP_PANEL_CHUNKS + MLP_WO_CHUNKS) {
    const int c = o - np * MLP_PANEL_CHUNKS - MLP_WO_CHUNKS, qp = c / MLP_W12_CHUNKS, cc = c - qp * MLP_W12_CHUNKS;
    const int r = cc >> 5, cp = cc & 31;
    const int ch = (cp & 16) | ((cp & 15) ^ (r & 15));
    int srow = qp * 64 + r;
    srow = srow < nq_rows ? srow : nq_rows - 1;
    const bf16_t* src = wq + (size_t)srow * 256 + (ch >> 2) * 32 + (ch & 3) * 4;
    const uint2 lo = *reinterpret_cast<const uint2*>(src), hi = *reinterpret_cast<const uint2*>(src + 16);
    out[o] = make_uint4(lo.x, lo.y, hi.x, hi.y);
    return;
  }
  if (o >= np * MLP_PANEL_CHUNKS) {
    const int c = o - np * MLP_PANEL_CHUNKS, wp = c / MLP_W12_CHUNKS, cc = c - wp * MLP_W12_CHUNKS;
    const int r = cc >> 5, cp = cc & 31;
    const int ch = (cp & 16) | ((cp & 15) ^ (r & 15));
    out[o] = wo ? *reinterpret_cast<const uint4*>(wo + (size_t)(wp * 64 + r) * 256 + ch * 8) : make_uint4(0, 0, 0, 0);
    return;
  }
  const int pn = o / MLP_PANEL_CHUNKS, c = o - pn * MLP_PANEL_CHUNKS;
  if (c < MLP_W12_CHUNKS) {
    const int r = c >> 5, cp = c & 31;
    const int ch = (cp & 16) | ((cp & 15) ^ (r & 15));
    const int srow = r < 32 ? pn * 32 + r : I + pn * 32 + (r - 32);
    const bf16_t* src = w12f + (size_t)srow * 256 + (ch >> 2) * 32 + (ch & 3) * 4;
    const uint2 lo = *reinterpret_cast<const uint2*>(src), hi = *reinterpret_cast<const uint2*>(src + 16);
// ... 16 lines not shown
  do {                                                                                                             \
    unsigned keep__;                                                                                               \
    asm volatile("s_mov_b32 %0, m0\n\t"                                                                            \
                 "s_mov_b32 m0, %6\n\ts_nop 0\n\tglobal_load_lds_dwordx4 %1, %5\n\t"                               \
                 "s_add_u32 m0, %6, 0x2000\n\ts_nop 0\n\tglobal_load_lds_dwordx4 %2, %5\n\t"                       \
                 "s_add_u32 m0, %6, 0x4000\n\ts_nop 0\n\tglobal_load_lds_dwordx4 %3, %5\n\t"                       \
                 "s_add_u32 m0, %6, 0x6000\n\ts_nop 0\n\tglobal_load_lds_dwordx4 %4, %5\n\t"                       \
                 "s_mov_b32 m0, %0"                                                                                \
                 : "=&s"(keep__)                                                                                   \
                 : "v"(lane16), "v"(lane16 + 8192u), "v"(lane16 + 16384u), "v"(lane16 + 24576u), "s"(src_), "s"(dst_) \
                 : "memory", "scc");                                                                               \
  } while (0)
#define MLP_GLDS_2(src_, dst_)                                                                                     \
  do {                                                                                                             \
    unsigned keep__;                                                                                               \
    asm volatile("s_mov_b32 %0, m0\n\t"                                                                            \
                 "s_mov_b32 m0, %4\n\ts_nop 0\n\tglobal_load_lds_dwordx4 %1, %3\n\t"                               \
                 "s_add_u32 m0, %4, 0x2000\n\ts_nop 0\n\tglobal_load_lds_dwordx4 %2, %3\n\t"                       \
                 "s_mov_b32 m0, %0"                                                                                \
                 : "=&s"(keep__)                                                                                   \
                 : "v"(lane16), "v"(lane16 + 8192u), "s"(src_), "s"(dst_)                                          \
                 : "memory", "scc");                                                                               \
  } while (0)
#ifdef MLP_STAMPS
#define MLP_STAMP()                                                                                                \
  do {                                                                                                             \
    if (p.stamps && blockIdx.x == 0 && (wave & 3) == 0 && lane == 0 && n_stamp < 64)                               \
      p.stamps[(wave >> 2) * 64 + n_stamp++] = (long long)__builtin_readcyclecounter();                            \
  } while (0)
#else
#define MLP_STAMP() do { (void)n_stamp; } while (0)
#endif

template <int TPB, int T1, int T2, bool GELU_FIRST, bool KEEL, bool FRONT, bool BACK>
__device__ __forceinline__ void mlp_wave(const MlpDev& p, uint4* l12, uint4* l3, uint4* hb, const float* gl, int tile, int wave, int lane,
                                         int P1F, int P2F, int& n_stamp) {
  constexpr int T1A = T1 > 0 ? T1 : 1, T2A = T2 > 0 ? T2 : 1;
  const int l15 = lane & 15, kq = lane >> 4;
  const int np = p.I / 32;
  const uint32_t lane16 = lane * 16;
  const uint32_t lds_l12 = (uint32_t)(uintptr_t)(__attribute__((address_space(3))) void*)l12;
  const uint32_t lds_l3 = (uint32_t)(uintptr_t)(__attribute__((address_space(3))) void*)l3;
#define GLDS_W12(pn_, buf_)                                                                                        \
  do {                                                                                                             \
    const uint4* src__ = p.pack + ((size_t)(pn_) * MLP_PANEL_CHUNKS + wave * 64);                                  \
    const uint32_t dst__ = lds_l12 + ((buf_) * MLP_W12_CHUNKS + wave * 64) * 16;                                   \
    MLP_GLDS_4(src__, dst__);                                                                                      \
  } while (0)
#define GLDS_W3(pn_, buf_)                                                                                         \
  do {                                                                                                             \
    const uint4* src__ = p.pack + ((size_t)(pn_) * MLP_PANEL_CHUNKS + MLP_W12_CHUNKS + wave * 64);                 \
    const uint32_t dst__ = lds_l3 + ((buf_) * MLP_W3_CHUNKS + wave * 64) * 16;                                     \
    MLP_GLDS_2(src__, dst__);                                                                                      \
  } while (0)

  const int tok0 = tile * (16 * TPB) + l15;
  typedef __attribute__((address_space(1))) char gchar;
  typedef __attribute__((address_space(1))) const char gcchar;
  gcchar* const gx = (gcchar*)p.x;
  gcchar* const gao = (gcchar*)p.ao;
  gchar* const gy = (gchar*)p.y;

  MLP_STAMP();
  __syncthreads();

  bf16x8 bfr[T1A][8];
  float rstd[T1A];
  if (FRONT) {
#define GLDS_WO(wp_, buf_)                                                                                         \
  do {                                                                                                             \
    const uint4* src__ = p.pack + ((size_t)np * MLP_PANEL_CHUNKS + (wp_) * MLP_W12_CHUNKS + wave * 64);            \
    const uint32_t dst__ = lds_l12 + ((buf_) * MLP_W12_CHUNKS + wave * 64) * 16;                                   \
    MLP_GLDS_4(src__, dst__);                                                                                      \
  } while (0)
    GLDS_WO(0, 0);
    bf16x8 abf[T1A][8];
#pragma unroll
    for (int j = 0; j < T1; ++j) {
      const int t = tok0 + 16 * (P1F + j);
      const int tc = t < p.M ? t : p.M - 1;
      const uint32_t aoff = ((uint32_t)tc * (uint32_t)p.ldao + kq * 8) * 2u;
#pragma unroll
      for (int s8 = 0; s8 < 8; ++s8) abf[j][s8] = *(const __attribute__((address_space(1))) bf16x8*)(gao + aoff + s8 * 64);
    }
    f32x4 facc[16][T1A];
    __builtin_amdgcn_s_waitcnt(0x0F70);
    __syncthreads();
#pragma unroll
    for (int wp = 0; wp < 4; ++wp) {
      if (wp + 1 < 4) GLDS_WO(wp + 1, (wp + 1) & 1);
      const uint4* img = l12 + (wp & 1) * MLP_W12_CHUNKS;
      bf16x8 a[2][4];
      if constexpr (T1 > 0) {
#pragma unroll
      for (int i = 0; i < 4; ++i) a[0][i] = MLP_LD12(img, i, 0);
#pragma unroll
      for (int s8 = 0; s8 < 8; ++s8) {
        if (s8 + 1 < 8) {
#pragma unroll
          for (int i = 0; i < 4; ++i) a[(s8 + 1) & 1][i] = MLP_LD12(img, i, s8 + 1);
        }
#pragma unroll
        for (int i = 0; i < 4; ++i)
#pragma unroll
          for (int j = 0; j < T1; ++j)
            facc[4 * wp + i][j] = __builtin_amdgcn_mfma_f32_16x16x32_bf16(a[s8 & 1][i], abf[j][s8],
                                                                           s8 ? facc[4 * wp + i][j] : (f32x4){0.f, 0.f, 0.f, 0.f}, 0, 0, 0);
        if (s8 + 1 < 8) __builtin_amdgcn_sched_group_barrier(0x100, 4, 0);
        __builtin_amdgcn_sched_group_barrier(0x008, 4 * T1A, 0);
        __builtin_amdgcn_sched_barrier(0);
      }
      }
      __builtin_amdgcn_s_waitcnt(0x0F70);
      __syncthreads();
    }
#undef GLDS_WO
    GLDS_W12(0, 0);
#pragma unroll
    for (int j = 0; j < T1; ++j) {
      const int t = tok0 + 16 * (P1F + j);
      const int tc = t < p.M ? t : p.M - 1;
      const uint32_t roff = ((uint32_t)tc * (uint32_t)p.ldx + kq * 4) * 2u;
      float ss = 0.f;
#pragma unroll
      for (int m = 0; m < 16; ++m) {
        facc[m][j] += p.front_alpha * cvt4(*(const __attribute__((address_space(1))) bf16x4*)(gx + roff + m * 32));
#pragma unroll
        for (int e = 0; e < 4; ++e) ss = fmaf(facc[m][j][e], facc[m][j][e], ss);
      }
      float scale = 1.0f;
      if (p.front_gain) {
        ss = quad16_sum(ss);
        scale = 1.0f / sqrtf(ss * (1.0f / 256.0f) + p.eps);
      }
      float ss2 = 0.f;
#pragma unroll
      for (int s8 = 0; s8 < 8; ++s8) {
        bf16x4 q[2];
#pragma unroll
        for (int u = 0; u < 2; ++u) {
          const int m = 2 * s8 + u;
          f32x4 v = facc[m][j];
          if (p.front_gain) {
            const f32x4 g = *reinterpret_cast<const f32x4*>(gl + 256 + m * 16 + kq * 4);
#pragma unroll
            for (int e = 0; e < 4; ++e) v[e] = v[e] * scale * g[e];
          }
          q[u] = (bf16x4){(bf16_t)v[0], (bf16_t)v[1], (bf16_t)v[2], (bf16_t)v[3]};
#pragma unroll
          for (int e = 0; e < 4; ++e) {
            const float r = (float)q[u][e];
            ss2 = fmaf(r, r, ss2);
          }
        }
        bfr[j][s8] = (bf16x8){q[0][0], q[0][1], q[0][2], q[0][3], q[1][0], q[1][1], q[1][2], q[1][3]};
      }
      ss2 = quad16_sum(ss2);
      rstd[j] = 1.0f / sqrtf(ss2 * (1.0f / 256.0f) + p.eps);
    }
  } else {
    GLDS_W12(0, 0);
#pragma unroll
    for (int j = 0; j < T1; ++j) {
      const int t = tok0 + 16 * (P1F + j);
      const int tc = t < p.M ? t : p.M - 1;
      const uint32_t xoff = ((uint32_t)tc * (uint32_t)p.ldx + kq * 4) * 2u;
#pragma unroll
      for (int s8 = 0; s8 < 8; ++s8) {
        const u32x2_t lo = *(const __attribute__((address_space(1))) u32x2_t*)(gx + xoff + s8 * 64);
        const u32x2_t hi = *(const __attribute__((address_space(1))) u32x2_t*)(gx + xoff + (s8 * 64 + 32));
        bfr[j][s8] = __builtin_bit_cast(bf16x8, (u32x4_t){lo.x, lo.y, hi.x, hi.y});
      }
    }
#pragma unroll
    for (int j = 0; j < T1; ++j) {
      float ss = 0.f;
#pragma unroll
      for (int s8 = 0; s8 < 8; ++s8)
#pragma unroll
        for (int e = 0; e < 8; ++e) {
          const float v = (float)bfr[j][s8][e];
          ss = fmaf(v, v, ss);
        }
      ss = quad16_sum(ss);
      rstd[j] = 1.0f / sqrtf(ss * (1.0f / 256.0f) + p.eps);
    }
  }
  f32x4 out[16][T2A];
#pragma unroll
  for (int m = 0; m < 16; ++m)
#pragma unroll
    for (int j = 0; j < T2; ++j) out[m][j] = (f32x4){0.f, 0.f, 0.f, 0.f};

  __builtin_amdgcn_s_waitcnt(0x0F70);
  __syncthreads();
  MLP_STAMP();

  for (int it = 0; it <= np; ++it) {
// ... 86 lines not shown
        for (int r = 0; r < 4; ++r) w3f[r] = __builtin_bit_cast(bf16x8, w3l[r * 16]);
  #pragma unroll
        for (int m = 0; m < 16; ++m) {
  #pragma unroll
          for (int j = 0; j < T2; ++j) out[m][j] = __builtin_amdgcn_mfma_f32_16x16x32_bf16(w3f[m & 3], hf[j], out[m][j], 0, 0, 0);
          if (m + 4 < 16) w3f[m & 3] = __builtin_bit_cast(bf16x8, w3l[(m + 4) * 16]);
          __builtin_amdgcn_sched_group_barrier(0x008, T2A, 0);
          if (m + 4 < 16) __builtin_amdgcn_sched_group_barrier(0x100, 1, 0);
          __builtin_amdgcn_sched_barrier(0);
        }
      }
    }
    if (it >= 4 && it < 8) MLP_STAMP();
    __builtin_amdgcn_s_waitcnt(0x0F70);
    __syncthreads();
    if (it >= 4 && it < 8) MLP_STAMP();
  }
  MLP_STAMP();

  uint4* const xres = l12;
  if (FRONT) {
#pragma unroll
    for (int j = 0; j < T1; ++j)
#pragma unroll
      for (int s8 = 0; s8 < 8; ++s8) xres[((P1F + j) * 8 + s8) * 64 + lane] = __builtin_bit_cast(uint4, bfr[j][s8]);
    __syncthreads();
  }

  bf16x8 xq[T2A][8];
  float rstdq[T2A];
#pragma unroll
  for (int j = 0; j < T2; ++j) {
    const int t = tok0 + 16 * (P2F + j);
    const bool tv = t < p.M;
    const int tc = tv ? t : p.M - 1;
    const uint32_t roff = ((uint32_t)tc * (uint32_t)p.ldx + kq * 4) * 2u;
    float ss = 0.f;
#pragma unroll
    for (int s8 = 0; s8 < 8; ++s8) {
      f32x4 rv0, rv1;
      if (FRONT) {
        const bf16x8 rb = __builtin_bit_cast(bf16x8, xres[((P2F + j) * 8 + s8) * 64 + lane]);
        rv0 = (f32x4){(float)rb[0], (float)rb[1], (float)rb[2], (float)rb[3]};
        rv1 = (f32x4){(float)rb[4], (float)rb[5], (float)rb[6], (float)rb[7]};
      } else {
        rv0 = cvt4(*(const __attribute__((address_space(1))) bf16x4*)(gx + roff + (2 * s8) * 32));
        rv1 = cvt4(*(const __attribute__((address_space(1))) bf16x4*)(gx + roff + (2 * s8 + 1) * 32));
      }
      out[2 * s8][j] += p.alpha * rv0;
      out[2 * s8 + 1][j] += p.alpha * rv1;
#pragma unroll
      for (int e = 0; e < 4; ++e) {
        ss = fmaf(out[2 * s8][j][e], out[2 * s8][j][e], ss);
        ss = fmaf(out[2 * s8 + 1][j][e], out[2 * s8 + 1][j][e], ss);
      }
    }
    float scale = 1.0f;
    if (KEEL) {
      ss = quad16_sum(ss);
      scale = 1.0f / sqrtf(ss * (1.0f / 256.0f) + p.eps);
    }
    const bool odd = kq & 1;
    const uint32_t yoff = ((uint32_t)tc * (uint32_t)p.ldy + (odd ? 16 + kq * 4 - 4 : kq * 4)) * 2u;
    float ssq = 0.f;
#pragma unroll
    for (int ip = 0; ip < 8; ++ip) {
      const int i0 = 2 * ip, i1 = 2 * ip + 1;
      f32x4 y0 = out[i0][j], y1 = out[i1][j];
// ... 12 lines not shown
        for (int e = 0; e < 4; ++e) {
          const float r0 = (float)q0[e], r1 = (float)q1[e];
          ssq = fmaf(r0, r0, ssq);
          ssq = fmaf(r1, r1, ssq);
        }
      }
      const uint4 ov = xchg16_pair(p0, p1);
      if (tv && !(p.debug & TTV_DBG_NO_STORES)) *(__attribute__((address_space(1))) u32x4_t*)(gy + yoff + ip * 64) = (u32x4_t){ov.x, ov.y, ov.z, ov.w};
    }
    if (BACK) {
      ssq = quad16_sum(ssq);
      rstdq[j] = 1.0f / sqrtf(ssq * (1.0f / 256.0f) + p.eps);
    }
  }
  MLP_STAMP();

  if (BACK) {
#define GLDS_WQ(qp_, buf_)                                                                                         \
  do {                                                                                                             \
    const uint4* src__ = p.pack + ((size_t)np * MLP_PANEL_CHUNKS + MLP_WO_CHUNKS + (qp_) * MLP_W12_CHUNKS + wave * 64); \
    const uint32_t dst__ = lds_l12 + ((buf_) * MLP_W12_CHUNKS + wave * 64) * 16;                                   \
    MLP_GLDS_4(src__, dst__);                                                                                      \
  } while (0)
    __syncthreads();
    GLDS_WQ(0, 0);
    gchar* const gq = (gchar*)p.qkv;
    gcchar* const grope = (gcchar*)p.rope_cs;
    f32x2 rc[4][T2A], rs[4][T2A];
    uint32_t qoff[T2A];
    bool qv[T2A];
#pragma unroll
    for (int j = 0; j < T2; ++j) {
      const int t = tok0 + 16 * (P2F + j);
      qv[j] = t < p.M;
      const int tc = qv[j] ? t : p.M - 1;
      qoff[j] = ((uint32_t)tc * (uint32_t)p.ldq + kq * 4) * 2u;
      gcchar* cs = grope + ((uint32_t)tc * 64u + kq * 2) * 4u;
#pragma unroll
      for (int i = 0; i < 4; ++i) {
        rc[i][j] = *(const __attribute__((address_space(1))) f32x2*)(cs + i * 32);
        rs[i][j] = *(const __attribute__((address_space(1))) f32x2*)(cs + 128 + i * 32);
      }
    }
    __builtin_amdgcn_s_waitcnt(0x0F70);
    __syncthreads();
    for (int qp = 0; qp < p.nqp; ++qp) {
      if (qp + 1 < p.nqp) GLDS_WQ(qp + 1, (qp + 1) & 1);
      const uint4* img = l12 + (qp & 1) * MLP_W12_CHUNKS;
      f32x4 qa[4][T2A];
      bf16x8 a[2][4];
#pragma unroll
      for (int i = 0; i < 4; ++i) a[0][i] = MLP_LD12(img, i, 0);
#pragma unroll
      for (int s8 = 0; s8 < 8; ++s8) {
        if (s8 + 1 < 8) {
#pragma unroll
          for (int i = 0; i < 4; ++i) a[(s8 + 1) & 1][i] = MLP_LD12(img, i, s8 + 1);
        }
#pragma unroll
        for (int i = 0; i < 4; ++i)
#pragma unroll
          for (int j = 0; j < T2; ++j)
            qa[i][j] = __builtin_amdgcn_mfma_f32_16x16x32_bf16(a[s8 & 1][i], xq[j][s8], s8 ? qa[i][j] : (f32x4){0.f, 0.f, 0.f, 0.f}, 0, 0, 0);
        if (s8 + 1 < 8) __builtin_amdgcn_sched_group_barrier(0x100, 4, 0);
        __builtin_amdgcn_sched_group_barrier(0x008, 4 * T2A, 0);
        __builtin_amdgcn_sched_barrier(0);
      }
      __builtin_amdgcn_s_waitcnt(0x0F70);
      __syncthreads();
      const int f_first = qp * 64;
      const bool rot = f_first < p.rope_q_end || (f_first >= p.rope_k_begin && f_first < p.rope_k_end);
#pragma unroll
      for (int j = 0; j < T2; ++j) {
        const bool odd = kq & 1;
        gchar* const qrow = gq + (qoff[j] - (uint32_t)(kq * 4) * 2u) + (uint32_t)(f_first + (odd ? 16 + kq * 4 - 4 : kq * 4)) * 2u;
#pragma unroll
        for (int ip = 0; ip < 2; ++ip) {
          uint2 pk[2];
#pragma unroll
          for (int u = 0; u < 2; ++u) {
            const int i = 2 * ip + u;
            f32x4 v = qa[i][j] * rstdq[j];
            if (rot)
              v = (f32x4){v[0] * rc[i][j].x - v[1] * rs[i][j].x, v[0] * rs[i][j].x + v[1] * rc[i][j].x,
                          v[2] * rc[i][j].y - v[3] * rs[i][j].y, v[2] * rs[i][j].y + v[3] * rc[i][j].y};
            const bf16x4 q = {(bf16_t)v[0], (bf16_t)v[1], (bf16_t)v[2], (bf16_t)v[3]};
            pk[u] = __builtin_bit_cast(uint2, q);
          }
          const uint4 ox = xchg16_pair(pk[0], pk[1]);
          const u32x4_t ov = {ox.x, ox.y, ox.z, ox.w};
          if (qv[j]) *(__attribute__((address_space(1))) u32x4_t*)(qrow + ip * 64) = ov;
        }
      }
    }
#undef GLDS_WQ
    MLP_STAMP();
  }
#undef GLDS_W12
#undef GLDS_W3
}

template <int TILES, bool KEEL, bool FRONT, bool BACK>
__global__ __launch_bounds__(512, 1) void k_mlp256(MlpDev p) {
  extern __shared__ __attribute__((aligned(16))) uint4 smem[];
  uint4* const l12 = smem;
  uint4* const l3 = smem + 2 * MLP_W12_CHUNKS;
  uint4* const hb = l3 + 2 * MLP_W3_CHUNKS;
  float* const gl = reinterpret_cast<float*>(hb + 2 * TILES * 64);
  if (threadIdx.x < 256) {
    gl[threadIdx.x] = p.post_gain ? p.post_gain[threadIdx.x] : 1.0f;
    gl[256 + threadIdx.x] = (FRONT && p.front_gain) ? p.front_gain[threadIdx.x] : 1.0f;
  }
  const int lane = threadIdx.x & 63;
  const int wave = __builtin_amdgcn_readfirstlane(threadIdx.x >> 6);
  int n_stamp = 0;
  const int tile = blockIdx.x;
  if constexpr (TILES == 9) {
    if (wave < 4) mlp_wave<9, 2, 0, false, KEEL, FRONT, BACK>(p, l12, l3, hb, gl, tile, wave, lane, 2 * wave, 0, n_stamp);
    else if (wave < 6) mlp_wave<9, 0, 3, false, KEEL, FRONT, BACK>(p, l12, l3, hb, gl, tile, wave, lane, 0, 3 * (wave - 4), n_stamp);
    else if (wave == 6) mlp_wave<9, 1, 1, false, KEEL, FRONT, BACK>(p, l12, l3, hb, gl, tile, wave, lane, 8, 6, n_stamp);
    else mlp_wave<9, 0, 2, false, KEEL, FRONT, BACK>(p, l12, l3, hb, gl, tile, wave, lane, 0, 7, n_stamp);
  } else {
    constexpr int NT = TILES / 4;
    constexpr int TA = NT - NT / 2;
    const int g0 = (wave & 3) * NT;
    if (wave < 4) mlp_wave<TILES, TA, NT - TA, false, KEEL, FRONT, BACK>(p, l12, l3, hb, gl, tile, wave, lane, g0, g0 + TA, n_stamp);
    else mlp_wave<TILES, NT - TA, TA, false, KEEL, FRONT, BACK>(p, l12, l3, hb, gl, tile, wave, lane, g0 + TA, g0, n_stamp);
  }
}
#undef MLP_LD12
#undef MLP_GLDS_4
#undef MLP_GLDS_2
#undef MLP_STAMP

bool ttvk_mlp_fused_supported(int dtype, int width, int inner) { return dtype == TTV_BF16 && width == 256 && inner % 32 == 0 && inner > 0; }

int64_t ttvk_mlp_pack_bytes(int inner, int next_qkv_rows) {
  if (inner <= 0 || inner % 32 != 0 || next_qkv_rows < 0) return 0;
  return ((int64_t)(inner / 32) * MLP_PANEL_CHUNKS + MLP_WO_CHUNKS + (int64_t)((next_qkv_rows + 63) / 64) * MLP_W12_CHUNKS) * 16;
}

int ttvk_mlp_pack(const void* w12_folded, const void* w3, const void* wo, const void* next_qkv_folded, int next_qkv_rows, int inner,
                  void* packed, hipStream_t s) {
  TTV_CHECK_ARG(w12_folded && w3 && packed, "mlp_pack: null buffer");
  TTV_CHECK_ARG(inner > 0 && inner % 32 == 0, "mlp_pack: inner %% 32");
  TTV_CHECK_ARG((next_qkv_folded != nullptr) == (next_qkv_rows > 0), "mlp_pack: next_qkv weight and row count must come together");
  TTV_CHECK_ARG(((uintptr_t)w12_folded % 16 == 0) && ((uintptr_t)packed % 16 == 0) && ((uintptr_t)wo % 16 == 0) &&
                    ((uintptr_t)next_qkv_folded % 16 == 0), "mlp_pack: 16-byte alignment");
  const int total = inner / 32 * MLP_PANEL_CHUNKS + MLP_WO_CHUNKS + (next_qkv_rows + 63) / 64 * MLP_W12_CHUNKS;
  hipLaunchKernelGGL(k_mlp_pack, dim3(ttv_cdiv(total, 256)), dim3(256), 0, s, (const bf16_t*)w12_folded, (const bf16_t*)w3,
                     (const bf16_t*)wo, (const bf16_t*)next_qkv_folded, next_qkv_rows, inner, (uint4*)packed);
  TTV_CHECK_LAUNCH("mlp_pack");
  return TTV_OK;
}

int ttvk_mlp_fused(const void* ao, int ldao, const float* front_gain, float front_alpha, const void* x, int ldx, const void* packed,
                   int inner, void* y, int ldy, const float* post_gain, float alpha, float eps, int M, const MlpNextQkv* nq, hipStream_t s) {
  if (M == 0) return TTV_OK;
  TTV_CHECK_ARG(x && packed && y, "mlp_fused: null buffer");
  TTV_CHECK_ARG(inner % 32 == 0 && ldx % 8 == 0 && ldy % 8 == 0 && (!ao || ldao % 8 == 0), "mlp_fused: inner %% 32, leading dims %% 8");
  TTV_CHECK_ARG(((uintptr_t)x % 16 == 0) && ((uintptr_t)packed % 16 == 0) && ((uintptr_t)y % 16 == 0) && ((uintptr_t)ao % 16 == 0),
                "mlp_fused: 16-byte alignment");
  MlpDev d;
  d.x = (const bf16_t*)x; d.ldx = ldx; d.pack = (const uint4*)packed; d.I = inner;
  d.ao = (const bf16_t*)ao; d.ldao = ldao; d.front_gain = front_gain; d.front_alpha = front_alpha;
  d.y = (bf16_t*)y; d.ldy = ldy; d.post_gain = post_gain; d.alpha = alpha; d.eps = eps; d.M = M; d.debug = g_ttv_debug; d.stamps = g_ttv_stamps;
  d.qkv = nullptr; d.ldq = 0; d.rope_cs = nullptr; d.nqp = 0; d.rope_q_end = d.rope_k_begin = d.rope_k_end = 0;
  if (nq) {
    TTV_CHECK_ARG(nq->qkv && nq->rope_cs && nq->rows > 0 && nq->rows % 64 == 0 && nq->ld >= nq->rows && nq->ld % 4 == 0 &&
                      (uintptr_t)nq->qkv % 8 == 0, "mlp_fused: bad next-qkv arguments (rows %% 64, ld %% 4, 8-byte aligned)");
    TTV_CHECK_ARG(nq->rope_q_end % 64 == 0 && nq->rope_k_begin % 64 == 0 && nq->rope_k_end % 64 == 0, "mlp_fused: rotary ranges must be whole heads");
    d.qkv = (bf16_t*)nq->qkv; d.ldq = nq->ld; d.rope_cs = nq->rope_cs; d.nqp = nq->rows / 64;
    d.rope_q_end = nq->rope_q_end; d.rope_k_begin = nq->rope_k_begin; d.rope_k_end = nq->rope_k_end;
  }
  const int cus = 256;
  int tiles = 4;
  long best = -1;
  for (int c = 1; c <= 3; ++c) {
    const long cost = (long)ttv_cdiv(ttv_cdiv(M, 64 * c), cus) * (16 + 19 * c);
    if (best < 0 || cost < best) { best = cost; tiles = 4 * c; }
  }
  if (!nq && !(g_ttv_debug & TTV_DBG_MLP_PAIRS_ONLY)) {
    const long cost9 = (long)ttv_cdiv(ttv_cdiv(M, 144), cus) * (16 + 14 * 3);
    if (cost9 < best) { best = cost9; tiles = 9; }
  }
  if ((g_ttv_debug & TTV_DBG_MLP_TILES9) && !nq) tiles = 9;
  if (g_ttv_debug & TTV_DBG_MLP_TILES8) tiles = 8;
  if (g_ttv_debug & TTV_DBG_MLP_TILES4) tiles = 4;
  d.n_tiles = ttv_cdiv(M, 16 * tiles);
  const int grid = d.n_tiles;
  const size_t smem = (size_t)(2 * MLP_W12_CHUNKS + 2 * MLP_W3_CHUNKS + 2 * tiles * 64) * sizeof(uint4) + 2048;
  TtvProfScope prof(TTV_KC_GEMM_GEGLU, s);
#define LAUNCH_MLP(TILES_, KEEL_, FRONT_, BACK_)                                                                    \
  do {                                                                                                              \
    (void)hipFuncSetAttribute((const void*)k_mlp256<TILES_, KEEL_, FRONT_, BACK_>, hipFuncAttributeMaxDynamicSharedMemorySize, (int)smem); \
    hipLaunchKernelGGL((k_mlp256<TILES_, KEEL_, FRONT_, BACK_>), dim3(grid), dim3(512), smem, s, d);                \
  } while (0)
#define LAUNCH_MLP_F(TILES_, KEEL_)                                                                                 \
  do {                                                                                                              \
    if (ao && nq) LAUNCH_MLP(TILES_, KEEL_, true, true);                                                            \
    else if (ao) LAUNCH_MLP(TILES_, KEEL_, true, false);                                                            \
    else LAUNCH_MLP(TILES_, KEEL_, false, false);                                                                   \
  } while (0)
#define LAUNCH_MLP_9(KEEL_)                                                                                         \
  do {                                                                                                              \
    if (ao) LAUNCH_MLP(9, KEEL_, true, false);                                                                      \
    else LAUNCH_MLP(9, KEEL_, false, false);                                                                        \
  } while (0)
  TTV_CHECK_ARG(!nq || ao, "mlp_fused: the next-qkv part needs the out_proj front (ttv_layer_tail_fused)");
  if (post_gain) {
    if (tiles == 9) LAUNCH_MLP_9(true); else if (tiles == 12) LAUNCH_MLP_F(12, true); else if (tiles == 8) LAUNCH_MLP_F(8, true); else LAUNCH_MLP_F(4, true);
  } else {
    if (tiles == 9) LAUNCH_MLP_9(false); else if (tiles == 12) LAUNCH_MLP_F(12, false); else if (tiles == 8) LAUNCH_MLP_F(8, false); else LAUNCH_MLP_F(4, false);
  }
#undef LAUNCH_MLP_9
#undef LAUNCH_MLP_F
#undef LAUNCH_MLP
  TTV_CHECK_LAUNCH("mlp_fused");
  return TTV_OK;
}
```

titok_video_amd/csrc/ttv_qkv256.inc:

```
#ifdef QKV_STAMPS
#define QK_STAMP_DECL unsigned long long qst_prev__ = 0, qst_acc__[8] = {0, 0, 0, 0, 0, 0, 0, 0}
#define QK_STAMP_START()                                                                                     \
  do {                                                                                                       \
    __builtin_amdgcn_sched_barrier(0);                                                                       \
    asm volatile("s_memtime %0\n\ts_waitcnt lgkmcnt(0)" : "=s"(qst_prev__)::"memory");                       \
    __builtin_amdgcn_sched_barrier(0);                                                                       \
  } while (0)
#define QK_STAMP(seg_)                                                                                       \
  do {                                                                                                       \
    unsigned long long t__;                                                                                  \
    __builtin_amdgcn_sched_barrier(0);                                                                       \
    asm volatile("s_memtime %0\n\ts_waitcnt lgkmcnt(0)" : "=s"(t__)::"memory");                              \
    __builtin_amdgcn_sched_barrier(0);                                                                       \
    qst_acc__[seg_] += t__ - qst_prev__;                                                                     \
    qst_prev__ = t__;                                                                                        \
  } while (0)
#else
#define QK_STAMP_DECL
#define QK_STAMP_START()
#define QK_STAMP(seg_)
#endif
typedef unsigned qk_u32x4 __attribute__((ext_vector_type(4)));
typedef unsigned qk_u32x2 __attribute__((ext_vector_type(2)));
template <bool PRENORM, bool FLOOR>
// ... 147 lines not shown
      __builtin_amdgcn_sched_group_barrier(0x008, 1, 0);                                                     \
      if (MODE_) { if ((ks__ & 1) || MODE_ != 2) __builtin_amdgcn_sched_group_barrier(0x002, 2, 0); else __builtin_amdgcn_sched_group_barrier(0x002, 4, 0); } \
      else if (PRENORM) __builtin_amdgcn_sched_group_barrier(0x002, 2, 0);                                   \
      __builtin_amdgcn_sched_barrier(0);                                                                     \
      if (MODE_ && (ks__ & 3) == 3) {                                                                        \
        QK_STORE_CHUNK(ks__ >> 2, pend_panel);                                                               \
        __builtin_amdgcn_sched_barrier(0);                                                                   \
      }                                                                                                      \
    }                                                                                                        \
    if (MODE_ == 0) {                                                                                        \
      if (PRENORM) {                                                                                         \
        float ss__ = ss0__ + ss1__;                                                                          \
        ss__ = pair32_sum(ss__);                                                                    \
        rstd = 1.0f / sqrtf(ss__ * (1.0f / 256.0f) + p.eps);                                                 \
      }                                                                                                      \
      _Pragma("unroll") for (int t__ = 0; t__ < 2; ++t__)                                                    \
        _Pragma("unroll") for (int g__ = 0; g__ < 4; ++g__)                                                  \
          _Pragma("unroll") for (int e__ = 0; e__ < 2; ++e__)                                                \
            rcs[t__][g__][e__] = make_float2(rcs[t__][g__][e__].x * rstd, rcs[t__][g__][e__].y * rstd);      \
    }                                                                                                        \
  } while (0)

#define QK_STEP(cur_, prev_, it_)                                                                            \
  do {                                                                                                       \
    const int it__ = (it_);                                                                                  \
    const int buf__ = (it__ - it0) & 1;                                                                      \
    int tile__, panel__;                                                                                     \
    if (FLOOR) {                                                                                             \
              \
      tile__ = fl_tile; panel__ = fl_panel;                                                                  \
      if (++fl_panel == n_panels) {                                                                          \
        ++fl_tile;                                                                                           \
        if (++fl_pos == p.tile_period) fl_pos = 0;                                                           \
        fl_panel = fl_pos < p.tile_run ? 0 : p.panel_lo;                                                     \
      }                                                                                                      \
    } else {                                                                                                 \
      tile__ = it__ / n_panels; panel__ = it__ - tile__ * n_panels;                                          \
    }                                                                                                        \
    if (tile__ != cur_tile) {                                                                                \
      cur_tile = tile__;                                                                                     \
       \
                                                                               \
        \
      const int ttile__ = FLOOR ? tile__ : p.tile_period ? (tile__ / p.tile_run) * p.tile_period + tile__ % p.tile_run : tile__; \
      const int t0__ = ttile__ * K256_TT + wave * 32;                                                        \
      int ntk__ = t0__ + r;                                                                                  \
      const bool nok__ = ntk__ < p.M;                                                                        \
      ntk__ = nok__ ? ntk__ : p.M - 1;                                                                       \
      const bf16_t* xr__ = X + (size_t)(p.x_rows ? p.x_rows[ntk__] : ntk__) * p.ldx + h * 8;                 \
      _Pragma("unroll") for (int ks__ = 0; ks__ < 16; ++ks__) bfr[ks__] = *reinterpret_cast<const bf16x8*>(xr__ + ks__ * 16); \
      uint2 nidp__ = make_uint2(0u, 0u);                                                                     \
      if (p.rope_ids) nidp__ = *reinterpret_cast<const uint2*>(p.rope_ids + 2 * (size_t)ntk__);              \
      if (pend == 2) QK_EPILOGUE(prev_, true, pend_panel); else if (pend == 1) QK_EPILOGUE(prev_, false, pend_panel); \
      pend = 0;                                                                                              \
       \
       \
       \
      _Pragma("unroll") for (int ks__ = 0; ks__ < 16; ++ks__) asm volatile("" : "+v"(bfr[ks__]));            \
      tk = ntk__; tok_ok = nok__; idp = nidp__;                                                              \
      wave_full = t0__ + 32 <= p.M;                                                                          \
      ytok = reinterpret_cast<char*>((bf16_t*)p.y + (size_t)tk * p.ldy) + h * 16;                            \
      rstd = 1.f;                                                                                            \
    }                                                                                                        \
    QK_STAMP(0);                                                                                             \
    if (it__ == it0) {                                                                                       \
      asm volatile("s_waitcnt vmcnt(0)" ::: "memory");                                                       \
      __syncthreads();                                                                                       \
// ... 1 lines not shown
    QK_STAMP(1);                                                                                             \
    const bool has_next__ = it__ + 1 < it1;                                                                  \
    const char* nsrc__ = QK_PANEL_SRC(FLOOR ? fl_panel : (it__ + 1) % n_panels);                             \
    const uint32_t ndst__ = QK_PANEL_DST(buf__ ^ 1);                                                         \
    const int f_first__ = panel__ * 64;                                                                      \
    const int rot__ = (f_first__ < p.rope_q_end || (f_first__ >= p.rope_k_begin && f_first__ < p.rope_k_end)) ? 2 : 1; \
    bool counted__ = false;                                                                                  \
    if (pend == 2) {                                                                                         \
      if (buf__) QK_BODY(cur_, prev_, 1, 2); else QK_BODY(cur_, prev_, 0, 2);                                \
      counted__ = wave_full && !(p.debug & TTV_DBG_NO_STORES);                                                               \
      QK_STAMP(2);                                                                                           \
    } else if (pend == 1) {                                                                                  \
      if (buf__) QK_BODY(cur_, prev_, 1, 1); else QK_BODY(cur_, prev_, 0, 1);                                \
      counted__ = wave_full && !(p.debug & TTV_DBG_NO_STORES);                                                               \
      QK_STAMP(2);                                                                                           \
    } else {                                                                                                 \
      if (buf__) QK_BODY(cur_, prev_, 1, 0); else QK_BODY(cur_, prev_, 0, 0);                                \
      QK_STAMP(3);                                                                                           \
    }                                                                                                        \
     \
    if (counted__) asm volatile("s_waitcnt vmcnt(3)" ::: "memory");                                          \
    else asm volatile("s_waitcnt vmcnt(0)" ::: "memory");                                                    \
    QK_STAMP(4);                                                                                             \
    __builtin_amdgcn_s_barrier();                                                                            \
    QK_STAMP(5);                                                                                             \
    pend = rot__;                                                                                            \
    pend_panel = panel__;                                                                                    \
  } while (0)

  f32x16 accA[2], accB[2];
  QK_STAMP_DECL;
  int fl_tile = 0, fl_panel = 0, fl_pos = 0;
  if (FLOOR) {
    const int full = p.tile_run * n_panels, wide = n_panels - p.panel_lo;
    const int per = full + (p.tile_period - p.tile_run) * wide;
    const int q = it0 / per;
    int rem = it0 - q * per;
    if (rem < full) { fl_pos = rem / n_panels; fl_panel = rem - fl_pos * n_panels; }
    else { rem -= full; fl_pos = p.tile_run + rem / wide; fl_panel = p.panel_lo + rem % wide; }
    fl_tile = q * p.tile_period + fl_pos;
  }
  {
    const char* src0 = QK_PANEL_SRC(FLOOR ? fl_panel : it0 % n_panels);
    const uint32_t dst0 = QK_PANEL_DST(0);
    QK_DMA_PIECE(dchunk0, 0, src0, dst0); QK_DMA_PIECE(dchunk0, 1, src0, dst0); QK_DMA_PIECE(dchunk0, 2, src0, dst0); QK_DMA_PIECE(dchunk0, 3, src0, dst0);
    QK_DMA_PIECE(dchunk0, 4, src0, dst0); QK_DMA_PIECE(dchunk0, 5, src0, dst0); QK_DMA_PIECE(dchunk0, 6, src0, dst0); QK_DMA_PIECE(dchunk0, 7, src0, dst0);
  }
  QK_STAMP_START();
  int it = it0;
  for (; it + 1 < it1; it += 2) {
    QK_STEP(accA, accB, it);
    QK_STEP(accB, accA, it + 1);
  }
  if (it < it1) {
    QK_STEP(accA, accB, it);
    if (pend == 2) QK_EPILOGUE(accA, true, pend_panel); else QK_EPILOGUE(accA, false, pend_panel);
  } else {
    if (pend == 2) QK_EPILOGUE(accB, true, pend_panel); else QK_EPILOGUE(accB, false, pend_panel);
  }
  QK_STAMP(6);
#ifdef QKV_STAMPS
  if (p.stamps && lb % 16 == 0 && lane == 0) {
    long long* dst = p.stamps + ((size_t)(lb / 16) * 4 + wave) * 8;
    for (int i = 0; i < 7; ++i) dst[i] = (long long)qst_acc__[i];
    dst[7] = it1 - it0;
  }
#endif
#undef QK_DMA_PIECE
#undef QK_PANEL_SRC
#undef QK_PANEL_DST
#undef QK_AFRAG
// ... 8 lines not shown
```

Before: 31960.

## Skip dead rows in last decoder layer and fuse decoder front kernels

Result: no change. 32380 (median of 3 runs) (+1.3%).

```diff
diff --git a/include/titok_hip.h b/include/titok_hip.h
--- a/include/titok_hip.h
+++ b/include/titok_hip.h
@@ -106,11 +106,17 @@
 int ttv_layer_tail_fused(const void* ao, int ldao, const float* attn_post_gain, float attn_alpha, const void* x, int ldx,
                          const void* mlp_packed, int inner, void* y, int ldy, const float* ffd_post_gain, float ffd_alpha, float eps,
                          int M, int width, int dtype, const ttv_next_qkv* next, void* stream);
+int ttv_layer_tail_fused_tiles(const void* ao, int ldao, const float* attn_post_gain, float attn_alpha, const void* x, int ldx,
+                               const void* mlp_packed, int inner, void* y, int ldy, const float* ffd_post_gain, float ffd_alpha, float eps,
+                               int M, int width, int dtype, int first_row, int period_rows, int run_rows, int periods, void* stream);
 
 int ttv_fill_const_rows(void* x, int dtype, int ld, const int32_t* rows_map, int rows, int width, const float* mask_token,
                         const float* gain, float eps, void* stream);
 int ttv_decoder_embed(const void* codes, int token_size, const void* w, const void* bias, const float* mask_token, const float* gain,
                       void* x, int dtype, int ld, const int32_t* rows_map, int rows, int width, float eps, void* stream);
+int ttv_decoder_front(const void* codes, int token_size, const void* w, const void* bias, const float* mask_token, const float* gain_t,
+                      const float* gain_p, void* x, int dtype, int ld, const int32_t* latent_rows, int n_latent, const int32_t* patch_rows,
+                      int n_patch, int width, float eps, void* stream);
 
 #define TTV_ATTN_GATE 1
 #define TTV_ATTN_PAIRED 2
@@ -535,7 +541,11 @@
   TTV_DBG_DEC_ALL_BLOCKS = 2097152,
   TTV_DBG_DEC_L0_NO_CONST = 4194304,
   TTV_DBG_ENC_LAST_QKV_ALL = 8388608,
-  TTV_DBG_PATCH_EMBED_UNFUSED = 16777216
+  TTV_DBG_PATCH_EMBED_UNFUSED = 16777216,
+  TTV_DBG_DEC_LAST_ALL_ROWS = 33554432,
+  TTV_DBG_ENC_LAST_COMPACT = 67108864,
+  TTV_DBG_DEC_FRONT_UNFUSED = 134217728,
+  TTV_DBG_DEC_LAST_QKV_ALL = 268435456
 };
 int ttv_debug_set(int flags);
 int ttv_debug_stamps(void* device_buffer);
diff --git a/titok_video_amd/_lib.py b/titok_video_amd/_lib.py
--- a/titok_video_amd/_lib.py
+++ b/titok_video_amd/_lib.py
@@ -43,6 +43,10 @@
 DBG_DEC_L0_NO_CONST = 4194304
 DBG_ENC_LAST_QKV_ALL = 8388608
 DBG_PATCH_EMBED_UNFUSED = 16777216
+DBG_DEC_LAST_ALL_ROWS = 33554432
+DBG_ENC_LAST_COMPACT = 67108864
+DBG_DEC_FRONT_UNFUSED = 134217728
+DBG_DEC_LAST_QKV_ALL = 268435456
 
 _HERE = os.path.dirname(os.path.abspath(__file__))
 LIB_PATH = switches.text("TTV_LIB_PATH") or os.path.join(_HERE, "libtitok_hip.so")
@@ -208,9 +212,12 @@
     "ttv_mlp_pack": (C.c_int, [vp, vp, vp, vp, C.c_int, C.c_int, C.c_int, C.c_int, vp, vp]),
     "ttv_layer_tail_fused": (C.c_int, [vp, C.c_int, vp, f32, vp, C.c_int, vp, C.c_int, vp, C.c_int, vp, f32, f32, C.c_int, C.c_int,
                                        C.c_int, vp, vp]),
+    "ttv_layer_tail_fused_tiles": (C.c_int, [vp, C.c_int, vp, f32, vp, C.c_int, vp, C.c_int, vp, C.c_int, vp, f32, f32, C.c_int, C.c_int,
+                                             C.c_int, C.c_int, C.c_int, C.c_int, C.c_int, vp]),
     "ttv_mlp_fused": (C.c_int, [vp, C.c_int, vp, C.c_int, vp, C.c_int, vp, f32, f32, C.c_int, C.c_int, C.c_int, vp]),
     "ttv_fill_const_rows": (C.c_int, [vp, C.c_int, C.c_int, vp, C.c_int, C.c_int, vp, vp, f32, vp]),
     "ttv_decoder_embed": (C.c_int, [vp, C.c_int, vp, vp, vp, vp, vp, C.c_int, C.c_int, vp, C.c_int, C.c_int, f32, vp]),
+    "ttv_decoder_front": (C.c_int, [vp, C.c_int, vp, vp, vp, vp, vp, vp, C.c_int, C.c_int, vp, C.c_int, vp, C.c_int, C.c_int, f32, vp]),
     "ttv_attention": (C.c_int, [vp, C.c_int, vp, C.c_int, vp, vp, C.c_int, C.c_int, C.c_int, C.c_int, C.c_int, C.c_int, vp]),
     "ttv_attention64": (C.c_int, [vp, C.c_int, vp, C.c_int, vp, vp, C.c_int, C.c_int, C.c_int, C.c_int, C.c_int, C.c_int, vp]),
     "ttv_rmsnorm_mx": (C.c_int, [vp, C.c_int, C.c_int, vp, C.c_int, C.c_int, vp, C.c_int, C.c_int, f32, vp, vp, vp, vp]),
diff --git a/titok_video_amd/csrc/ttv_api.hip b/titok_video_amd/csrc/ttv_api.hip
--- a/titok_video_amd/csrc/ttv_api.hip
+++ b/titok_video_amd/csrc/ttv_api.hip
@@ -26,6 +26,10 @@
 bool ttv_sw_attn_pipe() { static const bool v = ttv_env_flag("TTV_ATTN_PIPE", false); return v; }
 static bool sw_dec_l0_const() { static const bool v = ttv_env_flag("TTV_DEC_L0_CONST", true); return v; }
 static bool sw_enc_last_qkv_skip() { static const bool v = ttv_env_flag("TTV_ENC_LAST_QKV_SKIP", true); return v; }
+static bool sw_dec_last_patch_rows() { static const bool v = ttv_env_flag("TTV_DEC_LAST_PATCH_ROWS", true); return v; }
+static bool sw_dec_front_fused() { static const bool v = ttv_env_flag("TTV_DEC_FRONT_FUSED", true); return v; }
+static bool sw_dec_last_qkv_skip() { static const bool v = ttv_env_flag("TTV_DEC_LAST_QKV_SKIP", true); return v; }
+static bool sw_enc_last_in_place() { static const bool v = ttv_env_flag("TTV_ENC_LAST_IN_PLACE", true); return v; }
 float ttv_sw_attn_thr() { static const float v = ttv_env_float("TTV_ATTN_THR", 8.0f); return v; }
 thread_local int g_ttv_debug = 0;
 long long* g_ttv_stamps = nullptr;
@@ -166,7 +170,7 @@
 struct PreNormW { const float* gain; const void *w, *w_pn, *w_f8; const float* w_f8_scale; bool f8; };
 
 static int prenorm_proj(const LayerCtx& c, GemmEpilogue epi, const char* x, int rows, const PreNormW& p, int N, char* y, int y_image,
-                        bool rstd_valid, int tile_run = 0, int tile_period = 0, int panel_lo = 0) {
+                        bool rstd_valid, int tile_run = 0, int tile_period = 0, int panel_lo = 0, int panel_lo_run = 0) {
   const ttv_tower_dims* d = c.d;
   const TowerWs& ws = c.ws;
   const int dm = d->width, dt = d->dtype;
@@ -188,7 +192,7 @@
   a.row_scale = fold_gen ? ws.rstd : nullptr;
   a.x = fold ? x : ws.xn; a.w = fold ? p.w_pn : p.w;
   if (epi == EPI_QKV_ROPE) { a.rope_ids = c.b->rope_ids; a.rope_base = c.b->rope_ids ? c.b->rope_base : nullptr; }
-  a.tile_run = tile_run; a.tile_period = tile_period; a.panel_lo = panel_lo;
+  a.tile_run = tile_run; a.tile_period = tile_period; a.panel_lo = panel_lo; a.panel_lo_run = panel_lo_run;
   return ttvk_gemm(epi, a, c.s);
 }
 
@@ -238,6 +242,22 @@
   const ttv_batch* b = c.b;
   if (!sw_enc_last_qkv_skip() || (g_ttv_debug & TTV_DBG_ENC_LAST_QKV_ALL) || c.d->kind != TTV_ENCODER) return false;
   return qkv_tile_list_ok(c, lw, b->tokens_per_clip, b->max_patches_per_clip);
+}
+
+static bool one_geometry(const ttv_batch* b, int K, int P) {
+  return K > 0 && P > 0 && (int64_t)b->n_clips * K == b->sum_tokens && (int64_t)b->n_clips * P == b->sum_patches;
+}
+static bool dec_last_patch_rows_ok(const LayerCtx& c, const ttv_layer_weights& lw) {
+  const ttv_batch* b = c.b;
+  if (!sw_dec_last_patch_rows() || (g_ttv_debug & TTV_DBG_DEC_LAST_ALL_ROWS) || c.d->kind != TTV_DECODER) return false;
+  return qkv_tile_list_ok(c, lw, b->tokens_per_clip, b->max_patches_per_clip);
+}
+static bool enc_last_in_place_ok(const LayerCtx& c) {
+  const ttv_tower_dims* d = c.d;
+  const ttv_batch* b = c.b;
+  if (!sw_enc_last_in_place() || (g_ttv_debug & TTV_DBG_ENC_LAST_COMPACT) || d->kind != TTV_ENCODER) return false;
+  if (d->dtype != TTV_BF16 || d->width != 256 || c.split3) return false;
+  return b->tokens_per_clip % 64 == 0 && one_geometry(b, b->tokens_per_clip, b->max_patches_per_clip);
 }
 
 static int run_layers(const ttv_tower_dims* d, const ttv_tower_weights* w, const ttv_batch* b, const TowerWs& ws, hipStream_t s,
@@ -274,6 +294,7 @@
     xq_valid = false;
     const bool f8_qkv = rows_f8(dt, dm, lw.to_qkv_f8, lw.to_qkv_f8_scale, lw.to_qkv_mx, lw.to_qkv_pn);
     const bool f8_w12 = rows_f8(dt, dm, lw.w12_f8, lw.w12_f8_scale, lw.w12_mx, lw.w12_pn);
+    const bool dec_last_rows = pat_last && last && dt == TTV_BF16 && !ctx.pipe && dec_last_patch_rows_ok(ctx, lw);
     if (!qkv_ready) {
       const void* w_plain = (dt == TTV_BF16 && lw.to_qkv_qs) ? lw.to_qkv_qs : lw.to_qkv;
       const PreNormW qw = {lw.pre_ln, w_plain, lw.to_qkv_pn, lw.to_qkv_f8, lw.to_qkv_f8_scale, f8_qkv};
@@ -281,6 +302,9 @@
       else if (lat_last && last && !f8_qkv && enc_last_qkv_skip_ok(ctx, lw))
         TTV_TRY(prenorm_proj(ctx, EPI_QKV_ROPE, ws.x, L, qw, nq, ws.qkv, 0, rstd_valid, b->tokens_per_clip / 128,
                              (b->tokens_per_clip + b->max_patches_per_clip) / 128, 2 * dm / 64));
+      else if (dec_last_rows && !f8_qkv && sw_dec_last_qkv_skip() && !(g_ttv_debug & TTV_DBG_DEC_LAST_QKV_ALL))
+        TTV_TRY(prenorm_proj(ctx, EPI_QKV_ROPE, ws.x, L, qw, nq, ws.qkv, 0, rstd_valid, b->tokens_per_clip / 128,
+                             (b->tokens_per_clip + b->max_patches_per_clip) / 128, 0, 2 * dm / 64));
       else TTV_TRY(prenorm_proj(ctx, EPI_QKV_ROPE, ws.x, L, qw, nq, ws.qkv, s3img ? 2 : 0, rstd_valid));
     }
     const bool q_scaled = dt == TTV_BF16 && (lw.to_qkv_pn ? lw.qkv_q_prescaled != 0 : lw.to_qkv_qs != nullptr);
@@ -304,21 +328,27 @@
     char* cx = ws.x;
     char* cao = ws.ao;
     int Lc = L;
-    if (lat_now) {
+    static const bool use_fused_mlp = ttv_env_flag("TTV_FUSED_MLP", true);
+    static const bool use_fused_qkv = ttv_env_flag("TTV_FUSED_QKV", false);
+    const bool fused_tail = use_fused_mlp && ttvk_mlp_fused_supported(dt, dm, d->inner) && lw.mlp_pack;
+    MlpTiles runs = {};
+    const int seq_rows = b->tokens_per_clip + b->max_patches_per_clip;
+    if (lat_now && fused_tail && enc_last_in_place_ok(ctx)) runs = {0, seq_rows, b->tokens_per_clip, b->n_clips};
+    else if (dec_last_rows && fused_tail)
+      runs = {b->tokens_per_clip, seq_rows, b->max_patches_per_clip, b->n_clips};
+    if (lat_now && !runs.periods) {
       TTV_TRY(gather_rows(ws.x, ws.xl, b->latent_rows, b->sum_tokens, row_bytes, s));
       TTV_TRY(gather_rows(ws.ao, ws.aol, b->latent_rows, b->sum_tokens, row_bytes, s));
       cx = ws.xl; cao = ws.aol; Lc = b->sum_tokens;
       compacted = true;
     }
-    static const bool use_fused_mlp = ttv_env_flag("TTV_FUSED_MLP", true);
-    static const bool use_fused_qkv = ttv_env_flag("TTV_FUSED_QKV", false);
     const float alpha = keel_alpha(d, i);
-    if (use_fused_mlp && ttvk_mlp_fused_supported(dt, dm, d->inner) && lw.mlp_pack) {
+    if (fused_tail) {
       MlpNextQkv nx = {};
       const bool back = use_fused_qkv && !last && lw.mlp_pack_qkv_rows == nq && nq % 64 == 0 && dm % 64 == 0 && g % 64 == 0;
       if (back) { nx.qkv = ws.qkv; nx.ld = nq; nx.rope_cs = b->rope_cs; nx.rows = nq; nx.rope_q_end = dm; nx.rope_k_begin = 2 * dm; nx.rope_k_end = 2 * dm + g; }
       TTV_TRY(ttvk_mlp_fused(cao, dm, i == 0 ? nullptr : lw.attn_post_ln, alpha, cx, dm, lw.mlp_pack, d->inner, cx, dm, i == 0 ? nullptr : lw.ffd_post_ln,
-                             alpha, d->eps, Lc, back ? &nx : nullptr, s));
+                             alpha, d->eps, Lc, back ? &nx : nullptr, s, runs.periods ? &runs : nullptr));
       qkv_ready = back;
       continue;
     }
@@ -554,6 +584,19 @@
                         next ? &nx : nullptr, (hipStream_t)stream);
 }
 
+int ttv_layer_tail_fused_tiles(const void* ao, int ldao, const float* attn_post_gain, float attn_alpha, const void* x, int ldx,
+                               const void* mlp_packed, int inner, void* y, int ldy, const float* ffd_post_gain, float ffd_alpha, float eps,
+                               int M, int width, int dtype, int first_row, int period_rows, int run_rows, int periods, void* stream) {
+  if (!ttvk_mlp_fused_supported(dtype, width, inner)) {
+    ttv_set_error("layer_tail_fused_tiles: only bf16, width 256, inner %% 32 == 0");
+    return TTV_ERR_UNSUPPORTED;
+  }
+  TTV_CHECK_ARG(ao, "layer_tail_fused_tiles: null attention output");
+  const MlpTiles tl = {first_row, period_rows, run_rows, periods};
+  return ttvk_mlp_fused(ao, ldao, attn_post_gain, attn_alpha, x, ldx, mlp_packed, inner, y, ldy, ffd_post_gain, ffd_alpha, eps, M, nullptr,
+                        (hipStream_t)stream, &tl);
+}
+
 int ttv_fill_const_rows(void* x, int dtype, int ld, const int32_t* rows_map, int rows, int width, const float* mask_token,
                         const float* gain, float eps, void* stream) {
   TTV_CHECK_ARG(rows == 0 || (x && rows_map && mask_token && gain), "fill_const_rows: null buffer");
@@ -564,6 +607,15 @@
                       void* x, int dtype, int ld, const int32_t* rows_map, int rows, int width, float eps, void* stream) {
   TTV_CHECK_ARG(rows == 0 || (codes && w && bias && mask_token && gain && x && rows_map), "decoder_embed: null buffer");
   return ttvk_dec_embed(codes, token_size, w, bias, mask_token, gain, x, dtype, ld, rows_map, rows, width, eps, (hipStream_t)stream);
+}
+
+int ttv_decoder_front(const void* codes, int token_size, const void* w, const void* bias, const float* mask_token, const float* gain_t,
+                      const float* gain_p, void* x, int dtype, int ld, const int32_t* latent_rows, int n_latent, const int32_t* patch_rows,
+                      int n_patch, int width, float eps, void* stream) {
+  TTV_CHECK_ARG(n_latent == 0 || (codes && w && bias && mask_token && gain_t && x && latent_rows), "decoder_front: null buffer");
+  TTV_CHECK_ARG(n_patch == 0 || (x && patch_rows && mask_token && gain_p), "decoder_front: null buffer");
+  return ttvk_dec_front(codes, token_size, w, bias, mask_token, gain_t, gain_p, x, dtype, ld, latent_rows, n_latent, patch_rows, n_patch, width, eps,
+                        (hipStream_t)stream);
 }
 
 int ttv_attention(const void* qkvg, int ld, void* out, int ldo, const int32_t* cu_seqlens, const int32_t* qblocks, int n_qblocks,
@@ -746,8 +798,13 @@
   TTV_CHECK_ARG(ws.total <= workspace_bytes, "decoder_forward: workspace too small (%lld < %lld)", (long long)workspace_bytes, (long long)ws.total);
   const int dm = d->width, dt = d->dtype, P = b->sum_patches, pd = patch_dim(d);
 
-  TTV_TRY(ttvk_dec_embed(codes, d->token_size, w->proj_in_w, w->proj_in_b, w->mask_token, w->ln_pre_t, ws.x, dt, dm, b->latent_rows, b->sum_tokens, dm, d->eps, s));
-  TTV_TRY(ttvk_fill_const_rows(ws.x, dt, dm, b->patch_rows, P, dm, w->mask_token, w->ln_pre_p, d->eps, s));
+  if (sw_dec_front_fused() && !(g_ttv_debug & TTV_DBG_DEC_FRONT_UNFUSED)) {
+    TTV_TRY(ttvk_dec_front(codes, d->token_size, w->proj_in_w, w->proj_in_b, w->mask_token, w->ln_pre_t, w->ln_pre_p, ws.x, dt, dm, b->latent_rows,
+                           b->sum_tokens, b->patch_rows, P, dm, d->eps, s));
+  } else {
+    TTV_TRY(ttvk_dec_embed(codes, d->token_size, w->proj_in_w, w->proj_in_b, w->mask_token, w->ln_pre_t, ws.x, dt, dm, b->latent_rows, b->sum_tokens, dm, d->eps, s));
+    TTV_TRY(ttvk_fill_const_rows(ws.x, dt, dm, b->patch_rows, P, dm, w->mask_token, w->ln_pre_p, d->eps, s));
+  }
 
   TTV_TRY(run_layers(d, w, b, ws, s, l0));
 
diff --git a/titok_video_amd/csrc/ttv_elem.hip b/titok_video_amd/csrc/ttv_elem.hip
--- a/titok_video_amd/csrc/ttv_elem.hip
+++ b/titok_video_amd/csrc/ttv_elem.hip
@@ -361,12 +361,8 @@
 }
 
 template <typename T>
-__global__ __launch_bounds__(256) void k_fill_const_rows(T* __restrict__ x, int ld, const int* __restrict__ rows_map, int rows,
-                                                         int d, const float* __restrict__ mask_token,
-                                                         const float* __restrict__ gain, float eps) {
-  const int wave = threadIdx.x >> 6, lane = threadIdx.x & 63;
-  const int r = blockIdx.x * ROWS_PER_BLOCK + wave;
-  if (r >= rows) return;
+__device__ __forceinline__ void fill_const_row(T* __restrict__ x, int ld, const int* __restrict__ rows_map, int r, int lane, int d,
+                                               const float* __restrict__ mask_token, const float* __restrict__ gain, float eps) {
   const float m = round_to<T>(mask_token[0]);
   const float rstd = 1.0f / sqrtf(m * m + eps);
   T* q = x + (size_t)rows_map[r] * ld;
@@ -376,6 +372,15 @@
     Vec4<T>::store(q + c, o);
   }
 }
+template <typename T>
+__global__ __launch_bounds__(256) void k_fill_const_rows(T* __restrict__ x, int ld, const int* __restrict__ rows_map, int rows,
+                                                         int d, const float* __restrict__ mask_token,
+                                                         const float* __restrict__ gain, float eps) {
+  const int wave = threadIdx.x >> 6, lane = threadIdx.x & 63;
+  const int r = blockIdx.x * ROWS_PER_BLOCK + wave;
+  if (r >= rows) return;
+  fill_const_row<T>(x, ld, rows_map, r, lane, d, mask_token, gain, eps);
+}
 
 int ttvk_fill_const_rows(void* x, int dtype, int ld, const int* rows_map, int rows, int d, const float* mask_token,
                          const float* gain, float eps, hipStream_t s) {
@@ -391,13 +396,10 @@
 }
 
 template <typename T>
-__global__ __launch_bounds__(256) void k_dec_embed(const T* __restrict__ codes, int C, const T* __restrict__ w ,
-                                                   const T* __restrict__ bias, const float* __restrict__ mask_token,
-                                                   const float* __restrict__ gain, T* __restrict__ x, int ld,
-                                                   const int* __restrict__ rows_map, int rows, int d, float eps, T* __restrict__ hpre) {
-  const int wave = threadIdx.x >> 6, lane = threadIdx.x & 63;
-  const int r = blockIdx.x * ROWS_PER_BLOCK + wave;
-  if (r >= rows) return;
+__device__ __forceinline__ void dec_embed_row(const T* __restrict__ codes, int C, const T* __restrict__ w ,
+                                              const T* __restrict__ bias, const float* __restrict__ mask_token,
+                                              const float* __restrict__ gain, T* __restrict__ x, int ld,
+                                              const int* __restrict__ rows_map, int r, int lane, int d, float eps, T* __restrict__ hpre) {
   float cz[TTV_MAX_FSQ];
 #pragma unroll
   for (int c = 0; c < TTV_MAX_FSQ; ++c) cz[c] = c < C ? Cvt<T>::to_f(codes[(size_t)r * C + c]) : 0.f;
@@ -449,6 +451,47 @@
       Vec4<T>::store(q + c0, o);
     }
   }
+}
+template <typename T>
+__global__ __launch_bounds__(256) void k_dec_embed(const T* __restrict__ codes, int C, const T* __restrict__ w ,
+                                                   const T* __restrict__ bias, const float* __restrict__ mask_token,
+                                                   const float* __restrict__ gain, T* __restrict__ x, int ld,
+                                                   const int* __restrict__ rows_map, int rows, int d, float eps, T* __restrict__ hpre) {
+  const int wave = threadIdx.x >> 6, lane = threadIdx.x & 63;
+  const int r = blockIdx.x * ROWS_PER_BLOCK + wave;
+  if (r >= rows) return;
+  dec_embed_row<T>(codes, C, w, bias, mask_token, gain, x, ld, rows_map, r, lane, d, eps, hpre);
+}
+template <typename T>
+__global__ __launch_bounds__(256) void k_dec_front(const T* __restrict__ codes, int C, const T* __restrict__ w, const T* __restrict__ bias,
+                                                   const float* __restrict__ mask_token, const float* __restrict__ gain_t,
+                                                   const float* __restrict__ gain_p, T* __restrict__ x, int ld,
+                                                   const int* __restrict__ latent_rows, int n_latent, int latent_blocks,
+                                                   const int* __restrict__ patch_rows, int n_patch, int d, float eps) {
+  const int wave = threadIdx.x >> 6, lane = threadIdx.x & 63;
+  if ((int)blockIdx.x < latent_blocks) {
+    const int r = blockIdx.x * ROWS_PER_BLOCK + wave;
+    if (r < n_latent) dec_embed_row<T>(codes, C, w, bias, mask_token, gain_t, x, ld, latent_rows, r, lane, d, eps, nullptr);
+  } else {
+    const int r = (blockIdx.x - latent_blocks) * ROWS_PER_BLOCK + wave;
+    if (r < n_patch) fill_const_row<T>(x, ld, patch_rows, r, lane, d, mask_token, gain_p, eps);
+  }
+}
+
+int ttvk_dec_front(const void* codes, int C, const void* w, const void* bias, const float* mask_token, const float* gain_t, const float* gain_p,
+                   void* x, int dtype, int ld, const int* latent_rows, int n_latent, const int* patch_rows, int n_patch, int d, float eps,
+                   hipStream_t s) {
+  if (n_latent == 0 && n_patch == 0) return TTV_OK;
+  TTV_CHECK_ARG(C >= 1 && C <= TTV_MAX_TOKEN, "dec_front: token_size %d out of range", C);
+  TTV_CHECK_ARG(d % 4 == 0 && d <= 1024, "dec_front: width");
+  const int latent_blocks = ttv_cdiv(n_latent, ROWS_PER_BLOCK);
+  dim3 grid(latent_blocks + ttv_cdiv(n_patch, ROWS_PER_BLOCK));
+  if (dtype == TTV_BF16)
+    hipLaunchKernelGGL((k_dec_front<bf16_t>), grid, dim3(256), 0, s, (const bf16_t*)codes, C, (const bf16_t*)w, (const bf16_t*)bias, mask_token, gain_t, gain_p, (bf16_t*)x, ld, latent_rows, n_latent, latent_blocks, patch_rows, n_patch, d, eps);
+  else
+    hipLaunchKernelGGL((k_dec_front<float>), grid, dim3(256), 0, s, (const float*)codes, C, (const float*)w, (const float*)bias, mask_token, gain_t, gain_p, (float*)x, ld, latent_rows, n_latent, latent_blocks, patch_rows, n_patch, d, eps);
+  TTV_CHECK_LAUNCH("dec_front");
+  return TTV_OK;
 }
 
 int ttvk_dec_embed(const void* codes, int C, const void* w, const void* bias, const float* mask_token, const float* gain,
diff --git a/titok_video_amd/csrc/ttv_gemm.hip b/titok_video_amd/csrc/ttv_gemm.hip
--- a/titok_video_amd/csrc/ttv_gemm.hip
+++ b/titok_video_amd/csrc/ttv_gemm.hip
@@ -32,6 +32,7 @@
   int resid_rows;
   int tile_run, tile_period;
   int panel_lo;
+  int panel_lo_run;
 };
 
 struct PatchDst {
@@ -1859,14 +1860,19 @@
   if (dtype == TTV_BF16 && d.K == 256 && d.N % 8 == 0 && !((d.debug & TTV_DBG_K256_GENERAL) && !prenorm && EPI != EPI_STORE_PATCH)) {
     const int fo = (EPI == EPI_GEGLU) ? 32 : 64;
     const int n_panels = ttv_cdiv(d.N, fo), n_tiles = d.tile_period ? d.M / K256_TT / d.tile_period * d.tile_run : ttv_cdiv(d.M, K256_TT);
-    const int total = n_panels * n_tiles + (d.panel_lo ? d.M / K256_TT / d.tile_period * (d.tile_period - d.tile_run) * (n_panels - d.panel_lo) : 0);
+    const bool floor = d.panel_lo || d.panel_lo_run;
+    const int total = (n_panels - d.panel_lo_run) * n_tiles + (floor ? d.M / K256_TT / d.tile_period * (d.tile_period - d.tile_run) * (n_panels - d.panel_lo) : 0);
     static const int grid_env = ttv_env_int("TTV_K256_GRID", 0);
     int grid = total < 512 ? total : 512;
     if (grid_env > 0) grid = total < grid_env ? total : grid_env;
-    else if (d.panel_lo && total > 512) {
-      const int w = n_panels - d.panel_lo;
-      for (int ipb = 2; ipb <= w; ++ipb)
-        if (w % ipb == 0 && n_panels % ipb == 0 && total / ipb <= 512) { grid = total / ipb; break; }
+    else if (floor && total > 512) {
+      const int w = n_panels - d.panel_lo, wr = n_panels - d.panel_lo_run;
+      bool split = false;
+      for (int ipb = 2; ipb <= w && ipb <= wr; ++ipb)
+        if (w % ipb == 0 && wr % ipb == 0 && total / ipb <= 512) { grid = total / ipb; split = true; break; }
+      if (!split)
+        for (int g = 512; g >= 416; --g)
+          if (total % g == 0) { grid = g; break; }
     } else if (total > 512)
       for (int g = 512; g >= 416; --g)
         if (total % g == 0) { grid = g; break; }
@@ -1884,7 +1890,7 @@
           TTV_CHECK_LAUNCH("qkv256ws");
           return TTV_OK;
         }
-        if (d.panel_lo) {
+        if (floor) {
           if (prenorm) hipLaunchKernelGGL((k_qkv256<true, true>), dim3(grid), dim3(256), 0, s, d, n_panels, total);
           else hipLaunchKernelGGL((k_qkv256<false, true>), dim3(grid), dim3(256), 0, s, d, n_panels, total);
         } else if (prenorm) hipLaunchKernelGGL((k_qkv256<true, false>), dim3(grid), dim3(256), 0, s, d, n_panels, total);
@@ -2038,13 +2044,15 @@
   d.row_scale = a.row_scale;
   d.stamps = g_ttv_stamps;
   d.resid_rows = a.resid_rows;
-  d.tile_run = d.tile_period = d.panel_lo = 0;
+  d.tile_run = d.tile_period = d.panel_lo = d.panel_lo_run = 0;
   TTV_CHECK_ARG(a.panel_lo >= 0 && (!a.panel_lo || (a.tile_period && a.N % 64 == 0 && a.panel_lo < a.N / 64)),
+                "gemm: a panel floor goes with a tile list and leaves at least one 64-feature panel");
+  TTV_CHECK_ARG(a.panel_lo_run >= 0 && (!a.panel_lo_run || (a.tile_period && a.N % 64 == 0 && a.panel_lo_run < a.N / 64)),
                 "gemm: a panel floor goes with a tile list and leaves at least one 64-feature panel");
   if (a.tile_period) {
     TTV_CHECK_ARG(epi == EPI_QKV_ROPE && a.dtype == TTV_BF16 && a.K == 256 && a.tile_run > 0 && a.tile_run < a.tile_period &&
                   a.M % (K256_TT * a.tile_period) == 0, "gemm: a tile list is a to_qkv option of the bf16 K=256 kernel, M a whole number of periods");
-    d.tile_run = a.tile_run; d.tile_period = a.tile_period; d.panel_lo = a.panel_lo;
+    d.tile_run = a.tile_run; d.tile_period = a.tile_period; d.panel_lo = a.panel_lo; d.panel_lo_run = a.panel_lo_run;
   }
   TTV_CHECK_ARG(!a.row_scale || ((a.dtype == TTV_BF16 || a.split3) && (epi == EPI_STORE || epi == EPI_QKV_ROPE || epi == EPI_GEGLU)),
                 "gemm: row_scale is a STORE / QKV_ROPE / GEGLU option of the bf16 and the split-bf16 kernels");
diff --git a/titok_video_amd/csrc/ttv_kernels.h b/titok_video_amd/csrc/ttv_kernels.h
--- a/titok_video_amd/csrc/ttv_kernels.h
+++ b/titok_video_amd/csrc/ttv_kernels.h
@@ -15,6 +15,9 @@
                          const float* gain, float eps, hipStream_t s);
 int ttvk_dec_embed(const void* codes, int C, const void* w, const void* bias, const float* mask_token, const float* gain,
                    void* x, int dtype, int ld, const int* rows_map, int rows, int d, float eps, hipStream_t s);
+int ttvk_dec_front(const void* codes, int C, const void* w, const void* bias, const float* mask_token, const float* gain_t, const float* gain_p,
+                   void* x, int dtype, int ld, const int* latent_rows, int n_latent, const int* patch_rows, int n_patch, int d, float eps,
+                   hipStream_t s);
 int ttvk_fsq_forward(const ttv_fsq_params* p, const void* z, int z_dtype, int rows, void* codes, int codes_dtype, int* indices,
                      float* bounded, hipStream_t s);
 int ttvk_fsq_indices_to_codes(const ttv_fsq_params* p, const int* indices, int rows, void* codes, int codes_dtype, hipStream_t s);
@@ -82,6 +85,7 @@
   int resid_rows;
   int tile_run, tile_period;
   int panel_lo;
+  int panel_lo_run;
 };
 struct ClipPtrs { void* p[TTV_MAX_CLIPS_PER_LAUNCH]; };
 int ttvk_gemm(GemmEpilogue epi, const GemmArgs& a, hipStream_t s);
@@ -140,8 +144,12 @@
 int64_t ttvk_mlp_pack_bytes(int inner, int next_qkv_rows);
 int ttvk_mlp_pack(const void* w12_folded, const void* w3, const void* wo, const void* next_qkv_folded, int next_qkv_rows, int inner,
                   void* packed, hipStream_t s);
+struct MlpTiles {
+  int first_row, period_rows, run_rows, periods;
+};
 int ttvk_mlp_fused(const void* ao, int ldao, const float* front_gain, float front_alpha, const void* x, int ldx, const void* packed,
-                   int inner, void* y, int ldy, const float* post_gain, float alpha, float eps, int M, const MlpNextQkv* nq, hipStream_t s);
+                   int inner, void* y, int ldy, const float* post_gain, float alpha, float eps, int M, const MlpNextQkv* nq, hipStream_t s,
+                   const MlpTiles* tl = nullptr);
 
 int ttvk_l1_loss(void* const* recon, void* const* target, void* const* grad, const int* sizes, int n_clips, int total_clips, int dtype,
                  float* loss, hipStream_t s);
diff --git a/titok_video_amd/csrc/ttv_mlp.hip b/titok_video_amd/csrc/ttv_mlp.hip
--- a/titok_video_amd/csrc/ttv_mlp.hip
+++ b/titok_video_amd/csrc/ttv_mlp.hip
@@ -21,6 +21,7 @@
   float alpha, eps;
   int M, n_tiles, debug;
   long long* stamps;
+  int first_row, period_rows, run_blocks;
 };
 
 __global__ void k_mlp_pack(const bf16_t* __restrict__ w12f, const bf16_t* __restrict__ w3, const bf16_t* __restrict__ wo,
@@ -103,7 +104,7 @@
 #define MLP_STAMP() do { (void)n_stamp; } while (0)
 #endif
 
-template <int TPB, int T1, int T2, bool GELU_FIRST, bool KEEL, bool FRONT, bool BACK>
+template <int TPB, int T1, int T2, bool GELU_FIRST, bool KEEL, bool FRONT, bool BACK, bool MAP>
 __device__ __forceinline__ void mlp_wave(const MlpDev& p, uint4* l12, uint4* l3, uint4* hb, const float* gl, int tile, int wave, int lane,
                                          int P1F, int P2F, int& n_stamp) {
   constexpr int T1A = T1 > 0 ? T1 : 1, T2A = T2 > 0 ? T2 : 1;
@@ -125,7 +126,15 @@
     MLP_GLDS_2(src__, dst__);                                                                                      \
   } while (0)
 
-  const int tok0 = tile * (16 * TPB) + l15;
+  int row0 = 0, rend = 0;
+  if constexpr (MAP) {
+    const int run = tile / p.run_blocks;
+    const int run_first = p.first_row + run * p.period_rows;
+    row0 = run_first + (tile - run * p.run_blocks) * (16 * TPB);
+    rend = run_first + p.run_blocks * (16 * TPB);
+  }
+#define MLP_REND (MAP ? rend : p.M)
+  const int tok0 = (MAP ? row0 : tile * (16 * TPB)) + l15;
   typedef __attribute__((address_space(1))) char gchar;
   typedef __attribute__((address_space(1))) const char gcchar;
   gcchar* const gx = (gcchar*)p.x;
@@ -149,7 +158,7 @@
 #pragma unroll
     for (int j = 0; j < T1; ++j) {
       const int t = tok0 + 16 * (P1F + j);
-      const int tc = t < p.M ? t : p.M - 1;
+      const int tc = t < MLP_REND ? t : MLP_REND - 1;
       const uint32_t aoff = ((uint32_t)tc * (uint32_t)p.ldao + kq * 8) * 2u;
 #pragma unroll
       for (int s8 = 0; s8 < 8; ++s8) abf[j][s8] = *(const __attribute__((address_space(1))) bf16x8*)(gao + aoff + s8 * 64);
@@ -190,7 +199,7 @@
 #pragma unroll
     for (int j = 0; j < T1; ++j) {
       const int t = tok0 + 16 * (P1F + j);
-      const int tc = t < p.M ? t : p.M - 1;
+      const int tc = t < MLP_REND ? t : MLP_REND - 1;
       const uint32_t roff = ((uint32_t)tc * (uint32_t)p.ldx + kq * 4) * 2u;
       float ss = 0.f;
 #pragma unroll
@@ -234,7 +243,7 @@
 #pragma unroll
     for (int j = 0; j < T1; ++j) {
       const int t = tok0 + 16 * (P1F + j);
-      const int tc = t < p.M ? t : p.M - 1;
+      const int tc = t < MLP_REND ? t : MLP_REND - 1;
       const uint32_t xoff = ((uint32_t)tc * (uint32_t)p.ldx + kq * 4) * 2u;
 #pragma unroll
       for (int s8 = 0; s8 < 8; ++s8) {
@@ -387,8 +396,8 @@
 #pragma unroll
   for (int j = 0; j < T2; ++j) {
     const int t = tok0 + 16 * (P2F + j);
-    const bool tv = t < p.M;
-    const int tc = tv ? t : p.M - 1;
+    const bool tv = t < MLP_REND;
+    const int tc = tv ? t : MLP_REND - 1;
     const uint32_t roff = ((uint32_t)tc * (uint32_t)p.ldx + kq * 4) * 2u;
     float ss = 0.f;
 #pragma unroll
@@ -467,8 +476,8 @@
 #pragma unroll
     for (int j = 0; j < T2; ++j) {
       const int t = tok0 + 16 * (P2F + j);
-      qv[j] = t < p.M;
-      const int tc = qv[j] ? t : p.M - 1;
+      qv[j] = t < MLP_REND;
+      const int tc = qv[j] ? t : MLP_REND - 1;
       qoff[j] = ((uint32_t)tc * (uint32_t)p.ldq + kq * 4) * 2u;
       gcchar* cs = grope + ((uint32_t)tc * 64u + kq * 2) * 4u;
 #pragma unroll
@@ -533,36 +542,46 @@
   }
 #undef GLDS_W12
 #undef GLDS_W3
+#undef MLP_REND
 }
 
+#define MLP_BLOCK_BODY                                                                                             \
+  extern __shared__ __attribute__((aligned(16))) uint4 smem[];                                                        \
+  uint4* const l12 = smem;                                                                                            \
+  uint4* const l3 = smem + 2 * MLP_W12_CHUNKS;                                                                        \
+  uint4* const hb = l3 + 2 * MLP_W3_CHUNKS;                                                                           \
+  float* const gl = reinterpret_cast<float*>(hb + 2 * TILES * 64);                                                    \
+  if (threadIdx.x < 256) {                                                                                            \
+    gl[threadIdx.x] = p.post_gain ? p.post_gain[threadIdx.x] : 1.0f;                                                  \
+    gl[256 + threadIdx.x] = (FRONT && p.front_gain) ? p.front_gain[threadIdx.x] : 1.0f;                               \
+  }                                                                                                                   \
+  const int lane = threadIdx.x & 63;                                                                                  \
+  const int wave = __builtin_amdgcn_readfirstlane(threadIdx.x >> 6);                                                  \
+  int n_stamp = 0;                                                                                                    \
+  const int tile = blockIdx.x;                                                                                        \
+  if constexpr (TILES == 9) {                                                                                         \
+    if (wave < 4) mlp_wave<9, 2, 0, false, KEEL, FRONT, BACK, MAP>(p, l12, l3, hb, gl, tile, wave, lane, 2 * wave, 0, n_stamp);\
+    else if (wave < 6) mlp_wave<9, 0, 3, false, KEEL, FRONT, BACK, MAP>(p, l12, l3, hb, gl, tile, wave, lane, 0, 3 * (wave - 4), n_stamp);\
+    else if (wave == 6) mlp_wave<9, 1, 1, false, KEEL, FRONT, BACK, MAP>(p, l12, l3, hb, gl, tile, wave, lane, 8, 6, n_stamp);\
+    else mlp_wave<9, 0, 2, false, KEEL, FRONT, BACK, MAP>(p, l12, l3, hb, gl, tile, wave, lane, 0, 7, n_stamp);       \
+  } else {                                                                                                            \
+    constexpr int NT = TILES / 4;                                                                                     \
+    constexpr int TA = NT - NT / 2;                                                                                   \
+    const int g0 = (wave & 3) * NT;                                                                                   \
+    if (wave < 4) mlp_wave<TILES, TA, NT - TA, false, KEEL, FRONT, BACK, MAP>(p, l12, l3, hb, gl, tile, wave, lane, g0, g0 + TA, n_stamp);\
+    else mlp_wave<TILES, NT - TA, TA, false, KEEL, FRONT, BACK, MAP>(p, l12, l3, hb, gl, tile, wave, lane, g0 + TA, g0, n_stamp);\
+  }
 template <int TILES, bool KEEL, bool FRONT, bool BACK>
 __global__ __launch_bounds__(512, 1) void k_mlp256(MlpDev p) {
-  extern __shared__ __attribute__((aligned(16))) uint4 smem[];
-  uint4* const l12 = smem;
-  uint4* const l3 = smem + 2 * MLP_W12_CHUNKS;
-  uint4* const hb = l3 + 2 * MLP_W3_CHUNKS;
-  float* const gl = reinterpret_cast<float*>(hb + 2 * TILES * 64);
-  if (threadIdx.x < 256) {
-    gl[threadIdx.x] = p.post_gain ? p.post_gain[threadIdx.x] : 1.0f;
-    gl[256 + threadIdx.x] = (FRONT && p.front_gain) ? p.front_gain[threadIdx.x] : 1.0f;
-  }
-  const int lane = threadIdx.x & 63;
-  const int wave = __builtin_amdgcn_readfirstlane(threadIdx.x >> 6);
-  int n_stamp = 0;
-  const int tile = blockIdx.x;
-  if constexpr (TILES == 9) {
-    if (wave < 4) mlp_wave<9, 2, 0, false, KEEL, FRONT, BACK>(p, l12, l3, hb, gl, tile, wave, lane, 2 * wave, 0, n_stamp);
-    else if (wave < 6) mlp_wave<9, 0, 3, false, KEEL, FRONT, BACK>(p, l12, l3, hb, gl, tile, wave, lane, 0, 3 * (wave - 4), n_stamp);
-    else if (wave == 6) mlp_wave<9, 1, 1, false, KEEL, FRONT, BACK>(p, l12, l3, hb, gl, tile, wave, lane, 8, 6, n_stamp);
-    else mlp_wave<9, 0, 2, false, KEEL, FRONT, BACK>(p, l12, l3, hb, gl, tile, wave, lane, 0, 7, n_stamp);
-  } else {
-    constexpr int NT = TILES / 4;
-    constexpr int TA = NT - NT / 2;
-    const int g0 = (wave & 3) * NT;
-    if (wave < 4) mlp_wave<TILES, TA, NT - TA, false, KEEL, FRONT, BACK>(p, l12, l3, hb, gl, tile, wave, lane, g0, g0 + TA, n_stamp);
-    else mlp_wave<TILES, NT - TA, TA, false, KEEL, FRONT, BACK>(p, l12, l3, hb, gl, tile, wave, lane, g0 + TA, g0, n_stamp);
-  }
+  constexpr bool MAP = false;
+  MLP_BLOCK_BODY
 }
+template <int TILES, bool KEEL>
+__global__ __launch_bounds__(512, 1) void k_mlp256_tiles(MlpDev p) {
+  constexpr bool MAP = true, FRONT = true, BACK = false;
+  MLP_BLOCK_BODY
+}
+#undef MLP_BLOCK_BODY
 #undef MLP_LD12
 #undef MLP_GLDS_4
 #undef MLP_GLDS_2
@@ -590,8 +609,9 @@
 }
 
 int ttvk_mlp_fused(const void* ao, int ldao, const float* front_gain, float front_alpha, const void* x, int ldx, const void* packed,
-                   int inner, void* y, int ldy, const float* post_gain, float alpha, float eps, int M, const MlpNextQkv* nq, hipStream_t s) {
-  if (M == 0) return TTV_OK;
+                   int inner, void* y, int ldy, const float* post_gain, float alpha, float eps, int M, const MlpNextQkv* nq, hipStream_t s,
+                   const MlpTiles* tl) {
+  if (M == 0 || (tl && tl->periods == 0)) return TTV_OK;
   TTV_CHECK_ARG(x && packed && y, "mlp_fused: null buffer");
   TTV_CHECK_ARG(inner % 32 == 0 && ldx % 8 == 0 && ldy % 8 == 0 && (!ao || ldao % 8 == 0), "mlp_fused: inner %% 32, leading dims %% 8");
   TTV_CHECK_ARG(((uintptr_t)x % 16 == 0) && ((uintptr_t)packed % 16 == 0) && ((uintptr_t)y % 16 == 0) && ((uintptr_t)ao % 16 == 0),
@@ -608,21 +628,32 @@
     d.qkv = (bf16_t*)nq->qkv; d.ldq = nq->ld; d.rope_cs = nq->rope_cs; d.nqp = nq->rows / 64;
     d.rope_q_end = nq->rope_q_end; d.rope_k_begin = nq->rope_k_begin; d.rope_k_end = nq->rope_k_end;
   }
+  if (tl) {
+    TTV_CHECK_ARG(ao && !nq, "mlp_fused: a row-tile list needs the out_proj front and takes no next-qkv part");
+    TTV_CHECK_ARG(tl->periods > 0 && tl->run_rows > 0 && tl->run_rows % 64 == 0 && tl->first_row >= 0 &&
+                      (tl->periods == 1 || tl->period_rows >= tl->run_rows) &&
+                      (int64_t)tl->first_row + (int64_t)(tl->periods - 1) * tl->period_rows + tl->run_rows <= (int64_t)M,
+                  "mlp_fused: row-tile list (runs of a multiple of 64 rows, disjoint, inside the M rows)");
+  }
+  auto fits = [&](int t) { return !tl || tl->run_rows % (16 * t) == 0; };
+  auto blocks = [&](int t) { return tl ? tl->periods * (tl->run_rows / (16 * t)) : ttv_cdiv(M, 16 * t); };
   const int cus = 256;
   int tiles = 4;
   long best = -1;
   for (int c = 1; c <= 3; ++c) {
-    const long cost = (long)ttv_cdiv(ttv_cdiv(M, 64 * c), cus) * (16 + 19 * c);
+    if (!fits(4 * c)) continue;
+    const long cost = (long)ttv_cdiv(blocks(4 * c), cus) * (16 + 19 * c);
     if (best < 0 || cost < best) { best = cost; tiles = 4 * c; }
   }
-  if (!nq && !(g_ttv_debug & TTV_DBG_MLP_PAIRS_ONLY)) {
-    const long cost9 = (long)ttv_cdiv(ttv_cdiv(M, 144), cus) * (16 + 14 * 3);
+  if (!nq && !(g_ttv_debug & TTV_DBG_MLP_PAIRS_ONLY) && fits(9)) {
+    const long cost9 = (long)ttv_cdiv(blocks(9), cus) * (16 + 14 * 3);
     if (cost9 < best) { best = cost9; tiles = 9; }
   }
-  if ((g_ttv_debug & TTV_DBG_MLP_TILES9) && !nq) tiles = 9;
-  if (g_ttv_debug & TTV_DBG_MLP_TILES8) tiles = 8;
+  if ((g_ttv_debug & TTV_DBG_MLP_TILES9) && !nq && fits(9)) tiles = 9;
+  if ((g_ttv_debug & TTV_DBG_MLP_TILES8) && fits(8)) tiles = 8;
   if (g_ttv_debug & TTV_DBG_MLP_TILES4) tiles = 4;
-  d.n_tiles = ttv_cdiv(M, 16 * tiles);
+  d.n_tiles = blocks(tiles);
+  d.first_row = tl ? tl->first_row : 0; d.period_rows = tl ? tl->period_rows : 0; d.run_blocks = tl ? tl->run_rows / (16 * tiles) : 0;
   const int grid = d.n_tiles;
   const size_t smem = (size_t)(2 * MLP_W12_CHUNKS + 2 * MLP_W3_CHUNKS + 2 * tiles * 64) * sizeof(uint4) + 2048;
   TtvProfScope prof(TTV_KC_GEMM_GEGLU, s);
@@ -631,6 +662,11 @@
     (void)hipFuncSetAttribute((const void*)k_mlp256<TILES_, KEEL_, FRONT_, BACK_>, hipFuncAttributeMaxDynamicSharedMemorySize, (int)smem); \
     hipLaunchKernelGGL((k_mlp256<TILES_, KEEL_, FRONT_, BACK_>), dim3(grid), dim3(512), smem, s, d);                \
   } while (0)
+#define LAUNCH_MLP_TILES(TILES_, KEEL_)                                                                             \
+  do {                                                                                                              \
+    (void)hipFuncSetAttribute((const void*)k_mlp256_tiles<TILES_, KEEL_>, hipFuncAttributeMaxDynamicSharedMemorySize, (int)smem); \
+    hipLaunchKernelGGL((k_mlp256_tiles<TILES_, KEEL_>), dim3(grid), dim3(512), smem, s, d);                         \
+  } while (0)
 #define LAUNCH_MLP_F(TILES_, KEEL_)                                                                                 \
   do {                                                                                                              \
     if (ao && nq) LAUNCH_MLP(TILES_, KEEL_, true, true);                                                            \
@@ -643,13 +679,24 @@
     else LAUNCH_MLP(9, KEEL_, false, false);                                                                        \
   } while (0)
   TTV_CHECK_ARG(!nq || ao, "mlp_fused: the next-qkv part needs the out_proj front (ttv_layer_tail_fused)");
-  if (post_gain) {
+#define LAUNCH_MLP_MAP(KEEL_)                                                                                       \
+  do {                                                                                                              \
+    if (tiles == 9) LAUNCH_MLP_TILES(9, KEEL_);                                                                     \
+    else if (tiles == 12) LAUNCH_MLP_TILES(12, KEEL_);                                                              \
+    else if (tiles == 8) LAUNCH_MLP_TILES(8, KEEL_);                                                                \
+    else LAUNCH_MLP_TILES(4, KEEL_);                                                                                \
+  } while (0)
+  if (tl) {
+    if (post_gain) LAUNCH_MLP_MAP(true); else LAUNCH_MLP_MAP(false);
+  } else if (post_gain) {
     if (tiles == 9) LAUNCH_MLP_9(true); else if (tiles == 12) LAUNCH_MLP_F(12, true); else if (tiles == 8) LAUNCH_MLP_F(8, true); else LAUNCH_MLP_F(4, true);
   } else {
     if (tiles == 9) LAUNCH_MLP_9(false); else if (tiles == 12) LAUNCH_MLP_F(12, false); else if (tiles == 8) LAUNCH_MLP_F(8, false); else LAUNCH_MLP_F(4, false);
   }
+#undef LAUNCH_MLP_MAP
 #undef LAUNCH_MLP_9
 #undef LAUNCH_MLP_F
+#undef LAUNCH_MLP_TILES
 #undef LAUNCH_MLP
   TTV_CHECK_LAUNCH("mlp_fused");
   return TTV_OK;
diff --git a/titok_video_amd/csrc/ttv_qkv256.inc b/titok_video_amd/csrc/ttv_qkv256.inc
--- a/titok_video_amd/csrc/ttv_qkv256.inc
+++ b/titok_video_amd/csrc/ttv_qkv256.inc
@@ -203,7 +203,7 @@
       if (++fl_panel == n_panels) {                                                                          \
         ++fl_tile;                                                                                           \
         if (++fl_pos == p.tile_period) fl_pos = 0;                                                           \
-        fl_panel = fl_pos < p.tile_run ? 0 : p.panel_lo;                                                     \
+        fl_panel = fl_pos < p.tile_run ? p.panel_lo_run : p.panel_lo;                                        \
       }                                                                                                      \
     } else {                                                                                                 \
       tile__ = it__ / n_panels; panel__ = it__ - tile__ * n_panels;                                          \
@@ -271,11 +271,12 @@
   QK_STAMP_DECL;
   int fl_tile = 0, fl_panel = 0, fl_pos = 0;
   if (FLOOR) {
-    const int full = p.tile_run * n_panels, wide = n_panels - p.panel_lo;
+    const int wrun = n_panels - p.panel_lo_run, wide = n_panels - p.panel_lo;
+    const int full = p.tile_run * wrun;
     const int per = full + (p.tile_period - p.tile_run) * wide;
     const int q = it0 / per;
     int rem = it0 - q * per;
-    if (rem < full) { fl_pos = rem / n_panels; fl_panel = rem - fl_pos * n_panels; }
+    if (rem < full) { fl_pos = rem / wrun; fl_panel = p.panel_lo_run + rem - fl_pos * wrun; }
     else { rem -= full; fl_pos = p.tile_run + rem / wide; fl_panel = p.panel_lo + rem % wide; }
     fl_tile = q * p.tile_period + fl_pos;
   }
```
